# umautobots/LONER

Hardware: AMD Instinct MI355X
Metric: training rays/sec (higher is better)
Workload: dtype f32

## Files before the change

loner_amd/csrc/lnr_density.hip:

```cpp
#include <stdlib.h>

#include "lnr_density_api.h"
#include <vector>
#include <cstdlib>
#include <cstdio>

#include <mutex>
#include <unordered_map>

typedef float f32x4 __attribute__((ext_vector_type(4)));

#define LNR_ENC_BWD_MAX_BPG 2048

namespace {
struct WsNote { uint64_t layout; uint32_t epoch; bool ovf_zero; };
std::mutex g_ws_mutex;
std::unordered_map<const void*, WsNote> g_ws_notes;

uint64_t layout_signature(const LnrNetSpec* spec, int64_t cap) {
    uint64_t h = 1469598103934665603ull;
    auto mix = [&](const void* p, size_t n) { const unsigned char* b = (const unsigned char*)p; for (size_t i = 0; i < n; ++i) { h ^= b[i]; h *= 1099511628211ull; } };
    mix(spec, sizeof(LnrNetSpec));
    mix(&cap, sizeof(cap));
    return h;
}
void ws_bound_locked() { if (g_ws_notes.size() > 64) g_ws_notes.clear(); }
void ws_touch(const void* ws, uint64_t layout) {
    std::lock_guard<std::mutex> lock(g_ws_mutex);
    ws_bound_locked();
    auto it = g_ws_notes.find(ws);
    if (it == g_ws_notes.end()) g_ws_notes[ws] = WsNote{layout, 0u, false};
    else if (it->second.layout != layout) { it->second.layout = layout; it->second.ovf_zero = false; }
}
void ws_backward_begin(const void* ws, uint64_t layout, int* epoch, bool* clear) {
    std::lock_guard<std::mutex> lock(g_ws_mutex);
    ws_bound_locked();
    WsNote& n = g_ws_notes[ws];
    if (n.layout != layout) { n.layout = layout; n.ovf_zero = false; }
    *clear = !n.ovf_zero;
    n.ovf_zero = false;
    n.epoch = n.epoch >= 0x7FFFFFF0u ? 1u : n.epoch + 1u;
    if (n.epoch == 1u) *clear = true;
    *epoch = (int)n.epoch;
}
void ws_backward_done(const void* ws) {
    std::lock_guard<std::mutex> lock(g_ws_mutex);
    auto it = g_ws_notes.find(ws);
    if (it != g_ws_notes.end()) it->second.ovf_zero = true;
}
void ws_forget(const void* ws) {
    std::lock_guard<std::mutex> lock(g_ws_mutex);
    g_ws_notes.erase(ws);
}
}

#define LNR_SLAB_GROUPS 16
__device__ __forceinline__ void slab_fold_block(const float* __restrict__ slabs, int n_slabs, int n_mlp, float* __restrict__ grad, int overwrite, int block) {
    __shared__ float part[LNR_SLAB_GROUPS][64];
    const int px = threadIdx.x & 63, gy = threadIdx.x >> 6;
    const int i = block * 64 + px;
    const int per = (n_slabs + LNR_SLAB_GROUPS - 1) / LNR_SLAB_GROUPS;
    int b = gy * per;
    const int b_end = min(n_slabs, b + per);
    float s0 = 0.0f, s1 = 0.0f, s2 = 0.0f, s3 = 0.0f;
    if (i < n_mlp) {
        for (; b + 3 < b_end; b += 4) {
            s0 += slabs[(size_t)b * n_mlp + i]; s1 += slabs[(size_t)(b + 1) * n_mlp + i];
            s2 += slabs[(size_t)(b + 2) * n_mlp + i]; s3 += slabs[(size_t)(b + 3) * n_mlp + i];
        }
        for (; b < b_end; ++b) s0 += slabs[(size_t)b * n_mlp + i];
    }
    part[gy][px] = (s0 + s1) + (s2 + s3);
    __syncthreads();
    if (gy == 0 && i < n_mlp) {
        float s = 0.0f;
#pragma unroll
        for (int k = 0; k < LNR_SLAB_GROUPS; ++k) s += part[k][px];
        grad[i] = overwrite ? s : grad[i] + s;
    }
}
__global__ void __launch_bounds__(64 * LNR_SLAB_GROUPS)
reduce_slabs_kernel(const float* __restrict__ slabs, int n_slabs, int n_mlp, float* __restrict__ grad, int overwrite) {
    slab_fold_block(slabs, n_slabs, n_mlp, grad, overwrite, (int)blockIdx.x);
}

template <int PAIR>
__device__ __forceinline__ void reduce_one(long long* acc, uint2 r, uint32_t base) {
    if (PAIR) {
        uint32_t pi; float v0, v1;
        lnr_unpack_pair(r, pi, v0, v1);
        unsigned long long* a = reinterpret_cast<unsigned long long*>(acc) + 2 * pi;
        if (__builtin_expect(__builtin_fmaxf(__builtin_fabsf(v0), __builtin_fabsf(v1)) < 256.0f, 1)) {
            atomicAdd(a, (unsigned long long)lnr_to_fix_small(v0));
            atomicAdd(a + 1, (unsigned long long)lnr_to_fix_small(v1));
        } else {
            atomicAdd(a, (unsigned long long)lnr_to_fix(v0));
            atomicAdd(a + 1, (unsigned long long)lnr_to_fix(v1));
        }
    } else {
        const float v = __uint_as_float(r.y);
        if (v != 0.0f) atomicAdd(reinterpret_cast<unsigned long long*>(&acc[r.x - base]), (unsigned long long)lnr_to_fix(v));
    }
}
__device__ __forceinline__ void reduce_xpair(long long* acc, const LnrXRec& r) {
    uint32_t pi, t; float a0, a1, fx;
    lnr_unpack_xpair(r, pi, t, a0, a1, fx);
    const uint32_t pj = pi ^ ((2u << t) - 1u);
    long long q[4];
    lnr_xpair_fix(a0, a1, fx, q);
    unsigned long long* a = reinterpret_cast<unsigned long long*>(acc);
    atomicAdd(a + 2 * pi, (unsigned long long)q[0]);
    atomicAdd(a + 2 * pi + 1, (unsigned long long)q[1]);
    atomicAdd(a + 2 * pj, (unsigned long long)q[2]);
    atomicAdd(a + 2 * pj + 1, (unsigned long long)q[3]);
}

#ifdef LNR_PHASE_TIMING
__device__ unsigned long long lnr_reduce_phase_cycles[LNR_N_PHASES];
#endif
#define RED_SLICE (1 << LNR_SLICE_SHIFT)

typedef uint32_t red_u32x3 __attribute__((ext_vector_type(3), aligned(4)));
typedef uint32_t red_u32x4 __attribute__((ext_vector_type(4)));
__device__ __forceinline__ LnrXRec load_xrec_stream(const char* p) {
    const red_u32x3 v = __builtin_nontemporal_load(reinterpret_cast<const red_u32x3*>(p));
    LnrXRec r; r.a = v.x; r.b = v.y; r.c = v.z;
    return r;
}
__device__ __forceinline__ uint4 load_rec2_stream(const uint4* p) {
    const red_u32x4 v = __builtin_nontemporal_load(reinterpret_cast<const red_u32x4*>(p));
    return make_uint4(v.x, v.y, v.z, v.w);
}

template <int PAIR, int RED_U>
__device__ __forceinline__ void reduce_regions(long long* acc, const int* __restrict__ wave_counts, const char* __restrict__ wave_regions, int n_regions,
                                               uint32_t region_bytes, bool xp, uint32_t base, int lane) {
    for (int r0 = 0; r0 < n_regions; r0 += 64) {
        const int nq = min(64, n_regions - r0);
        const int my_n = lane < nq ? wave_counts[r0 + lane] : 0;
        const char* round_regions = wave_regions + (size_t)r0 * region_bytes;
        if (xp) {
            LnrXRec cur[RED_U][2], nxt[RED_U][2];
            auto loadx = [&](int q0, LnrXRec out[RED_U][2]) {
#pragma unroll
                for (int u = 0; u < RED_U; ++u) {
                    const int q = q0 + u < nq ? q0 + u : nq - 1;
                    const int n = __builtin_amdgcn_readlane(my_n, q);
                    const char* rg = round_regions + (size_t)q * region_bytes;
                    out[u][0] = load_xrec_stream(rg + (lane < n ? lane : 0) * 12);
                    out[u][1] = load_xrec_stream(rg + (lane + 64 < n ? lane + 64 : 0) * 12);
                }
            };
            loadx(0, nxt);
            for (int q0 = 0; q0 < nq; q0 += RED_U) {
#pragma unroll
                for (int u = 0; u < RED_U; ++u) { cur[u][0] = nxt[u][0]; cur[u][1] = nxt[u][1]; }
                if (q0 + RED_U < nq) loadx(q0 + RED_U, nxt);
#pragma unroll
                for (int u = 0; u < RED_U; ++u) {
                    const int n = q0 + u < nq ? __builtin_amdgcn_readlane(my_n, q0 + u < 64 ? q0 + u : 63) : 0;
                    if (lane < n) reduce_xpair(acc, cur[u][0]);
                    if (lane + 64 < n) reduce_xpair(acc, cur[u][1]);
                }
            }
            unsigned long long more = __ballot(my_n > 128);
            while (more) {
                const int q = __builtin_ctzll(more);
                more &= more - 1ull;
                const int n = __builtin_amdgcn_readlane(my_n, q);
                const char* rg = round_regions + (size_t)q * region_bytes;
                for (int off = 128; off < n; off += 64 * 4) {
                    LnrXRec r[4];
#pragma unroll
                    for (int u = 0; u < 4; ++u) { const int k = off + 64 * u + lane; r[u] = load_xrec_stream(rg + (size_t)(k < n ? k : n - 1) * 12); }
#pragma unroll
                    for (int u = 0; u < 4; ++u) if (off + 64 * u + lane < n) reduce_xpair(acc, r[u]);
                }
            }
            continue;
        }
        uint4 cur[RED_U], nxt[RED_U];
        auto load4 = [&](int q0, uint4 out[RED_U]) {
#pragma unroll
            for (int u = 0; u < RED_U; ++u) {
                const int q = q0 + u < nq ? q0 + u : nq - 1;
                const int n = __builtin_amdgcn_readlane(my_n, q);
                out[u] = load_rec2_stream(reinterpret_cast<const uint4*>(round_regions + (size_t)q * region_bytes) + (2 * lane < n ? lane : 0));
            }
        };
        load4(0, nxt);
        for (int q0 = 0; q0 < nq; q0 += RED_U) {
#pragma unroll
            for (int u = 0; u < RED_U; ++u) cur[u] = nxt[u];
            if (q0 + RED_U < nq) load4(q0 + RED_U, nxt);
#pragma unroll
            for (int u = 0; u < RED_U; ++u) {
                const int n = q0 + u < nq ? __builtin_amdgcn_readlane(my_n, q0 + u < 64 ? q0 + u : 63) : 0;
                if (2 * lane < n) reduce_one<PAIR>(acc, make_uint2(cur[u].x, cur[u].y), base);
                if (2 * lane + 1 < n) reduce_one<PAIR>(acc, make_uint2(cur[u].z, cur[u].w), base);
            }
        }
        unsigned long long more = __ballot(my_n > 128);
        while (more) {
            const int q = __builtin_ctzll(more);
            more &= more - 1ull;
            const int n = __builtin_amdgcn_readlane(my_n, q);
            const uint2* rg = reinterpret_cast<const uint2*>(round_regions + (size_t)q * region_bytes);
            for (int off = 128; off < n; off += 128 * 4) {
                uint4 r[4];
#pragma unroll
                for (int u = 0; u < 4; ++u) { const int k = off + 128 * u + 2 * lane; r[u] = load_rec2_stream(reinterpret_cast<const uint4*>(rg) + (k < n ? k : 0) / 2); }
#pragma unroll
                for (int u = 0; u < 4; ++u) {
                    const int k = off + 128 * u + 2 * lane;
                    if (k < n) reduce_one<PAIR>(acc, make_uint2(r[u].x, r[u].y), base);
                    if (k + 1 < n) reduce_one<PAIR>(acc, make_uint2(r[u].z, r[u].w), base);
                }
            }
        }
    }
}

struct RedLevel { uint64_t lo, hi; };
__device__ __forceinline__ RedLevel red_level(const LnrNetSpec& spec, int l) {
    RedLevel r;
    r.lo = (uint64_t)spec.level_offset[l] * spec.n_features;
    r.hi = r.lo + (uint64_t)spec.level_size[l] * spec.n_features;
    return r;
}

template <int PAIR, int RED_U, int MINW>
__global__ void __launch_bounds__(1024, MINW)
table_grad_reduce_split_kernel(const LnrNetSpec spec, const void* __restrict__ regions_v, const RegionPlan plan, const int* __restrict__ counts, int bpg,
                               int maxo, long long* __restrict__ ovf) {
    extern __shared__ long long acc[];
    constexpr int slice = RED_SLICE, shift = LNR_SLICE_SHIFT;
    int b = blockIdx.x, l = 0, span = 0;
    int64_t my_ovf = 0;
    RedLevel lv;
    for (;; ++l) {
        lv = red_level(spec, l);
        span = (int)(((lv.hi - 1) >> shift) - (lv.lo >> shift)) + 1;
        const int n = plan.split[l] > 1 ? span * plan.split[l] : 0;
        if (b < n) break;
        b -= n;
        my_ovf += (int64_t)(lv.hi - lv.lo);
    }
    const int parts = plan.split[l], local = b / parts, part = b % parts;
    const uint32_t base = ((uint32_t)(lv.lo >> shift) + (uint32_t)local) << shift;
    const uint32_t region_bytes = plan.bytes[l];
    if (region_bytes == 0u) return;
#pragma unroll
    for (int i = threadIdx.x; i < slice; i += 1024) acc[i] = 0ll;
    __syncthreads();
    const int lane = threadIdx.x & 63, wave = __builtin_amdgcn_readfirstlane(threadIdx.x >> 6);
    const int per_part = (bpg + parts - 1) / parts, part_first = part * per_part, part_n = min(per_part, bpg - part_first);
    const int per_wave = (part_n + 15) / 16, first = part_first + wave * per_wave, n_regions = min(per_wave, part_first + part_n - first);
    if (n_regions > 0)
        reduce_regions<PAIR, RED_U>(acc, counts + ((size_t)l * maxo + local) * bpg + first,
                                    reinterpret_cast<const char*>(regions_v) + plan.off[l] + ((size_t)local * bpg + first) * (size_t)region_bytes, n_regions,
                                    region_bytes, PAIR && plan.xp[l] != 0, base, lane);
    __syncthreads();
#pragma unroll
    for (int k = 0; k < slice / 1024; ++k) {
        const int i = threadIdx.x + k * 1024;
        const uint64_t gi = (uint64_t)base + i;
        const long long q = acc[i];
        if (q != 0ll && gi >= lv.lo && gi < lv.hi) atomicAdd(reinterpret_cast<unsigned long long*>(ovf + my_ovf + (int64_t)(gi - lv.lo)), (unsigned long long)q);
    }
}

template <int PAIR, int RED_U, int MINW>
__global__ void __launch_bounds__(1024, MINW)
table_grad_reduce2_kernel(const LnrNetSpec spec, const void* __restrict__ regions_v, const RegionPlan plan, const int* __restrict__ counts, int bpg,
                          int maxo, long long* __restrict__ ovf, const int* __restrict__ ovf_flag, int epoch, float* __restrict__ grad_table,
                          int64_t n_table_floats, int overwrite, const float* __restrict__ slabs, int n_slabs, int n_mlp, float* __restrict__ grad_mlp) {
    extern __shared__ long long acc[];
    const int slab_blocks = slabs != nullptr ? (n_mlp + 63) / 64 : 0;
    const int owner_blocks = (int)gridDim.x - slab_blocks;
    if ((int)blockIdx.x >= owner_blocks) {
        slab_fold_block(slabs, n_slabs, n_mlp, grad_mlp, overwrite, (int)blockIdx.x - owner_blocks);
        return;
    }
    const int o = owner_blocks - 1 - (int)blockIdx.x;
    constexpr int slice = RED_SLICE, shift = LNR_SLICE_SHIFT;
    const uint32_t base = (uint32_t)o << shift;
    PHASE_INIT();
#pragma unroll
    for (int i = threadIdx.x; i < slice; i += 1024) acc[i] = 0ll;
    __syncthreads();
    PHASE(0);
    const int lane = threadIdx.x & 63, wave = __builtin_amdgcn_readfirstlane(threadIdx.x >> 6);
    constexpr int nwaves = 16;
    int64_t ovf_off = 0;
    for (int l = 0; l < spec.n_levels; ++l) {
        const RedLevel lv = red_level(spec, l);
        const uint64_t lo = lv.lo, hi = lv.hi;
        const int64_t my_ovf = ovf_off;
        ovf_off += (int64_t)(hi - lo);
        if (hi <= base || lo >= (uint64_t)base + slice) continue;
        if (plan.split[l] > 1 || ovf_flag[l] == epoch) {
            long long v[slice / 1024];
#pragma unroll
            for (int k = 0; k < slice / 1024; ++k) {
                const uint64_t gi = (uint64_t)base + threadIdx.x + k * 1024;
                v[k] = (gi >= lo && gi < hi) ? ovf[my_ovf + (int64_t)(gi - lo)] : 0ll;
            }
#pragma unroll
            for (int k = 0; k < slice / 1024; ++k) {
                if (v[k] != 0ll) {
                    acc[threadIdx.x + k * 1024] += v[k];
                    ovf[my_ovf + (int64_t)((uint64_t)base + threadIdx.x + k * 1024 - lo)] = 0ll;
                }
            }
            __syncthreads();
            PHASE(1);
        }
        const int local = o - (int)(lo >> shift);
        if (local < 0 || local >= maxo) continue;
        const uint32_t region_bytes = plan.bytes[l];
        if (region_bytes == 0u || plan.split[l] > 1) continue;
        const int per_wave = (bpg + nwaves - 1) / nwaves;
        const int first = wave * per_wave;
        const int n_regions = min(per_wave, bpg - first);
        if (n_regions > 0)
            reduce_regions<PAIR, RED_U>(acc, counts + ((size_t)l * maxo + local) * bpg + first,
                                        reinterpret_cast<const char*>(regions_v) + plan.off[l] + ((size_t)local * bpg + first) * (size_t)region_bytes, n_regions,
                                        region_bytes, PAIR && plan.xp[l] != 0, base, lane);
        PHASE(3);
    }
    __syncthreads();
    PHASE(5);
    {
        float g[slice / 1024];
#pragma unroll
        for (int k = 0; k < slice / 1024; ++k) {
            const int64_t gi = (int64_t)base + threadIdx.x + k * 1024;
            g[k] = (!overwrite && gi < n_table_floats) ? grad_table[gi] : 0.0f;
        }
#pragma unroll
        for (int k = 0; k < slice / 1024; ++k) {
            const int64_t gi = (int64_t)base + threadIdx.x + k * 1024;
            const long long q = acc[threadIdx.x + k * 1024];
            if (gi < n_table_floats && (overwrite || q != 0ll)) grad_table[gi] = g[k] + (float)((double)q * (1.0 / (double)LNR_FIX_SCALE));
        }
    }
    PHASE(6);
    PHASE_FLUSH(lnr_reduce_phase_cycles, 0);
}

struct Layout {
    int64_t m_pad;
    int n_groups, bpg, maxo, shift, nown, n_split;
    RegionPlan plan;
    size_t off_status, off_feat, off_wide, off_dfeat, off_dxl, off_dpts, off_rayacc, off_slabs, off_ovf, off_counts, off_regions, total;
};

static size_t align256(size_t v) { return (v + 255) & ~(size_t)255; }

static Layout make_layout(const LnrNetSpec* spec, int64_t n_points, const DensityRoute& route) {
    Layout L;
    L.m_pad = (n_points + 63) / 64 * 64;
    if (L.m_pad < 64) L.m_pad = 64;
#ifndef LNR_PLANE_SKEW
#define LNR_PLANE_SKEW 1088
#endif
    if (LNR_PLANE_SKEW > 0 && (L.m_pad * (int64_t)sizeof(float)) % 65536 == 0) L.m_pad += LNR_PLANE_SKEW;
    const bool hash = spec->encoding == LNR_ENC_HASHGRID;
    L.n_groups = hash ? spec->n_levels : 1;
    L.shift = LNR_SLICE_SHIFT;
    const int64_t n_table = spec->n_params - spec->n_mlp_params;
    L.nown = (int)((n_table + (1 << L.shift) - 1) >> L.shift);
    int64_t bpg = (n_points + LNR_ENC_BWD_BLOCK * LNR_BATCHES_PER_WG - 1) / (LNR_ENC_BWD_BLOCK * LNR_BATCHES_PER_WG);
    if (bpg < 1) bpg = 1;
    if (bpg > LNR_ENC_BWD_MAX_BPG) bpg = LNR_ENC_BWD_MAX_BPG;
    bpg = (bpg + 3) & ~(int64_t)3;
    L.bpg = (int)bpg;
    L.maxo = 1;
    size_t ovf_total = 0;
    uint64_t region_total = 0;
    for (int l = 0; l < LNR_MAX_LEVELS; ++l) { L.plan.off[l] = 0; L.plan.bytes[l] = 0; L.plan.xp[l] = 0; L.plan.split[l] = 1; L.plan.binned[l] = 0; }
    L.n_split = 0;
    if (hash) {
        const int F = spec->n_features;
        for (int pass = 0; pass < 2; ++pass) {
            if (pass == 1 && region_total <= LNR_REGION_BUDGET) break;
            const double shrink = pass == 0 ? 1.0 : (double)LNR_REGION_BUDGET / (double)region_total;
            region_total = 0; ovf_total = 0; L.maxo = 1; L.n_split = 0;
            for (int l = 0; l < spec->n_levels; ++l) {
                ovf_total += (size_t)spec->level_size[l] * F;
                const uint64_t lo = (uint64_t)spec->level_offset[l] * F, hi = lo + (uint64_t)spec->level_size[l] * F;
                const int span = (int)(((hi - 1) >> L.shift) - (lo >> L.shift)) + 1;
                if (span > L.maxo) L.maxo = span;
                const bool xp = lnr_level_can_use_xpairs(*spec, l, LNR_XPAIR_SCALE_MIN);
                L.plan.xp[l] = xp ? 1 : 0;
                double r = (double)n_points * 8.0 * (F >= 2 ? F / 2.0 : 1.0) / (double)span / (double)L.bpg;
                if (xp) r *= 0.5;
                else if (spec->level_scale[l] < LNR_COMBINE_SCALE_MAX) r *= LNR_COMBINE_FILL;
                const double recs = (r * (xp ? LNR_REGION_HEADROOM_XP : LNR_REGION_HEADROOM) + LNR_REGION_SLACK) * shrink;
                uint64_t bytes = (uint64_t)(recs * (xp ? 12.0 : 8.0));
                const double bin_fill = (double)LNR_ENC_BWD_BLOCK * 8.0 * (xp ? 0.5 * 12.0 : 8.0) / (double)span;
                const bool binned = F >= 2 && spec->level_hashed[l] != 0 && span <= LNR_BIN_MAX_OWNERS && bin_fill <= 0.5 * LNR_BIN_BYTES + 8.0 &&
                                    LNR_ENC_BWD_BLOCK == 512 && shrink == 1.0;
                L.plan.binned[l] = binned ? 1 : 0;
                if (binned) bytes += LNR_BIN_BYTES + 128;
                bytes = (bytes + 255u) & ~(uint64_t)255u;
                int parts = spec->level_hashed[l] == 0 ? LNR_REDUCE_SPLIT : 1;
                while (parts > 1 && L.bpg / parts < 16) parts >>= 1;
                L.plan.split[l] = (uint8_t)(parts < 1 ? 1 : parts);
// ... 247 lines not shown
    ws_forget(workspace);
    if (hipMemsetAsync(workspace, 0, LNR_WORKSPACE_STATUS_BYTES, (hipStream_t)stream) != hipSuccess) {
        lnr_set_error("lnr_density_workspace_init: hipMemsetAsync failed");
        return LNR_ERR_LAUNCH;
    }
    return LNR_OK;
}

extern "C" int lnr_density_workspace_release(void* workspace) {
    LNR_REQUIRE(workspace != nullptr, "lnr_density_workspace_release: null workspace");
    ws_forget(workspace);
    return LNR_OK;
}

extern "C" int lnr_density_forward(const LnrNetSpec* spec, const float* params, const float* pts, int64_t n_points,
                                   const float* rays, const float* z, int32_t n_rays, int32_t n_samples,
                                   const int32_t* n_rays_dev, float* sigma, void* workspace, size_t workspace_bytes, void* stream) {
    int rc = check_spec(spec, "lnr_density_forward");
    if (rc) return rc;
    if (n_points == 0 && (pts != nullptr || n_rays == 0)) return LNR_OK;
    PointSrc src; MlpPoints mp;
    rc = make_src(&src, &mp, pts, n_points, rays, z, n_rays, n_samples, n_rays_dev, "lnr_density_forward");
    if (rc) return rc;
    const int64_t cap = mp.n_points;
    if (cap == 0) return LNR_OK;
    LNR_REQUIRE(params && sigma && workspace, "lnr_density_forward: null params/sigma/workspace");
    const DensityRoute route = lnr_route(spec, cap, false);
    const Layout L = make_layout(spec, cap, route);
    LNR_REQUIRE(L.m_pad * (spec->n_features > 4 ? spec->n_features : 4) < (1ll << 30),
                "lnr_density_forward: too many points per call for 32-bit plane offsets (padded n_points * max(n_features, 4) must be < 2^30)");
    if (workspace_bytes < L.off_dfeat) {
        lnr_set_error("lnr_density_forward: workspace %zu < %zu (lnr_density_workspace_forward)", workspace_bytes, L.off_dfeat);
        return LNR_ERR_WORKSPACE;
    }
    if (route.kind == LNR_ROUTE_UNSUPPORTED) return route_unsupported(spec, route, "lnr_density_forward");
    hipStream_t st = (hipStream_t)stream;
    ws_touch(workspace, layout_signature(spec, cap));
    float* feat = (float*)((char*)workspace + L.off_feat);
    mp.clip_flag = reinterpret_cast<int32_t*>((char*)workspace + L.off_status) + LNR_STATUS_CLIPPED;
    if (!route.fused_enc) {
        LnrProfScope prof("encode_forward", st);
        rc = lnr_encode_forward(spec, params, &src, cap, feat, L.m_pad, spec->precision == LNR_PREC_F16, st);
    }
    if (rc) return rc;
    LNR_CHECK_LAUNCH("lnr_density_forward(encode)");
    LnrProfScope prof_mlp("mlp_forward", st);
    const MlpArgs a{spec, &route, params, feat, L.m_pad, &mp, sigma, nullptr, nullptr, nullptr, 0, 0, &src, nullptr, (char*)workspace + L.off_wide, st};
    const char* what;
    switch (route.kind) {
        case LNR_ROUTE_WIDE: rc = lnr_mlp_fwd_wide(a); what = "lnr_density_forward(mlp 256 x n)"; break;
        case LNR_ROUTE_F16_FAST: case LNR_ROUTE_F16_FREQ: case LNR_ROUTE_F16_GEN: rc = lnr_mlp_fwd_f16(a); what = "lnr_density_forward(mlp f16)"; break;
        case LNR_ROUTE_BF3: rc = lnr_mlp_fwd_bf3(a); what = "lnr_density_forward(mlp bf16x3)"; break;
        default: rc = mlp_fwd_ht(a); what = "lnr_density_forward(mlp)"; break;
    }
    if (rc) return rc;
    LNR_CHECK_LAUNCH(what);
    return LNR_OK;
}

extern "C" int lnr_density_backward(const LnrNetSpec* spec, const float* params, const float* pts, int64_t n_points,
                                    const float* rays, const float* z, int32_t n_rays, int32_t n_samples,
                                    const int32_t* n_rays_dev, const float* d_sigma, float* grad_params, float* d_pts, float* d_rays,
                                    int32_t reuse_features, int32_t flags, void* workspace, size_t workspace_bytes, void* input_grad_event,
                                    void* stream) {
    int rc = check_spec(spec, "lnr_density_backward");
    if (rc) return rc;
    auto empty_batch = [&]() -> int {
        if (input_grad_event != nullptr && hipEventRecord((hipEvent_t)input_grad_event, (hipStream_t)stream) != hipSuccess) {
            lnr_set_error("lnr_density_backward: hipEventRecord failed");
            return LNR_ERR_LAUNCH;
        }
        return LNR_OK;
    };
    if (n_points == 0 && (pts != nullptr || n_rays == 0)) return empty_batch();
    PointSrc src; MlpPoints mp;
    rc = make_src(&src, &mp, pts, n_points, rays, z, n_rays, n_samples, n_rays_dev, "lnr_density_backward");
    if (rc) return rc;
    const int64_t cap = mp.n_points;
    if (cap == 0) return empty_batch();
    LNR_REQUIRE(params && d_sigma && workspace, "lnr_density_backward: null argument");
    LNR_REQUIRE(grad_params || d_pts || d_rays, "lnr_density_backward: nothing to compute (no grad_params, d_pts or d_rays)");
    const DensityRoute route = lnr_route(spec, cap, true);
    const Layout L = make_layout(spec, cap, route);
    LNR_REQUIRE(L.m_pad * (spec->n_features > 4 ? spec->n_features : 4) < (1ll << 30),
                "lnr_density_backward: too many points per call for 32-bit plane offsets (padded n_points * max(n_features, 4) must be < 2^30)");
    if (workspace_bytes < L.total) {
        lnr_set_error("lnr_density_backward: workspace %zu < %zu (lnr_density_workspace)", workspace_bytes, L.total);
        return LNR_ERR_WORKSPACE;
    }
    if (route.kind == LNR_ROUTE_UNSUPPORTED) return route_unsupported(spec, route, "lnr_density_backward");
    hipStream_t st = (hipStream_t)stream;
    char* ws = (char*)workspace;
    float* feat = (float*)(ws + L.off_feat);
    float* dfeat = (float*)(ws + L.off_dfeat);
    float* dxl = (float*)(ws + L.off_dxl);
    float* slabs = (float*)(ws + L.off_slabs);
    long long* ovf = (long long*)(ws + L.off_ovf);
    int* counts = (int*)(ws + L.off_counts);
    void* regions = (void*)(ws + L.off_regions);
    const bool hash = spec->encoding == LNR_ENC_HASHGRID;
    RegionPlan rplan = L.plan;
    if (flags & LNR_BWD_TABLE_ATOMICS)
        for (int l = 0; l < LNR_MAX_LEVELS; ++l) rplan.bytes[l] = 0;
    if (!(flags & LNR_BWD_BINS))
        for (int l = 0; l < LNR_MAX_LEVELS; ++l) rplan.binned[l] = 0;
    const bool want_grad = grad_params != nullptr;

    const bool fused_freq = route.fused_enc;
    if (!reuse_features && !fused_freq) {
        LnrProfScope prof("encode_forward", st);
        rc = lnr_encode_forward(spec, params, &src, cap, feat, L.m_pad, spec->precision == LNR_PREC_F16, st);
        if (rc) return rc;
        LNR_CHECK_LAUNCH("lnr_density_backward(encode)");
    }
    LNR_REQUIRE(!(d_rays && pts), "lnr_density_backward: d_rays needs the rays form");
    LNR_REQUIRE(!(d_rays && d_pts), "lnr_density_backward: pass d_pts or d_rays, not both");
    const bool ray_accum = d_rays != nullptr && hash && (n_samples % 64 == 0);
    float* d_pts_eff = d_pts;
    if (d_rays && !ray_accum) d_pts_eff = (float*)(ws + L.off_dpts);
    const int want_dfeat = ((hash && want_grad) || d_pts_eff != nullptr || ray_accum) ? 1 : 0;
    {
    LnrProfScope prof("mlp_backward", st);
    const MlpArgs a{spec, &route, params, feat, L.m_pad, &mp, nullptr, d_sigma, dfeat, slabs, want_dfeat, want_grad ? 1 : 0, &src, d_pts_eff, ws + L.off_wide, st};
    switch (route.kind) {
        case LNR_ROUTE_WIDE: rc = lnr_mlp_bwd_wide(a); break;
        case LNR_ROUTE_F16_FAST: case LNR_ROUTE_F16_FREQ: case LNR_ROUTE_F16_GEN: rc = lnr_mlp_bwd_f16(a); break;
        case LNR_ROUTE_BF3: rc = lnr_mlp_bwd_bf3(a); break;
        case LNR_ROUTE_REGS: rc = mlp_bwd_regs(a); break;
        default: rc = mlp_bwd_ht(a); break;
    }
    }
    if (rc) return rc;
    LNR_CHECK_LAUNCH("lnr_density_backward(mlp)");
    float* grad_table = want_grad ? grad_params + spec->n_mlp_params : nullptr;
    int* ovf_flag = reinterpret_cast<int32_t*>(ws + L.off_status) + LNR_STATUS_OVF_LEVEL0;
    int epoch = 0;
    const bool uses_ovf = hash && want_grad;
    if (uses_ovf) {
        bool clear = false;
        ws_backward_begin(workspace, layout_signature(spec, cap), &epoch, &clear);
        if (clear && (hipMemsetAsync(ovf, 0, L.off_counts - L.off_ovf, st) != hipSuccess ||
                      hipMemsetAsync(ovf_flag, 0, LNR_MAX_LEVELS * sizeof(int32_t), st) != hipSuccess)) {
            lnr_set_error("lnr_density_backward: hipMemsetAsync failed");
            return LNR_ERR_LAUNCH;
        }
    } else {
        ws_touch(workspace, layout_signature(spec, cap));
    }
    const bool fold_in_reduce = want_grad && hash && L.nown > 0 && !(flags & LNR_BWD_DEFER_WEIGHT_FOLD);
    ReduceCtx rctx{spec, regions, counts, ovf, ovf_flag, epoch, grad_table, rplan, L.bpg, L.maxo, L.shift, spec->n_params - spec->n_mlp_params,
                   (flags & LNR_BWD_TABLE_ATOMICS) ? 0 : L.n_split, (flags & LNR_BWD_OVERWRITE_GRAD) ? 1 : 0,
                   fold_in_reduce ? slabs : nullptr, route.n_slabs, spec->n_mlp_params, grad_params};
    if (want_dfeat && !fused_freq) {
        rc = lnr_encode_backward(spec, params, &src, cap, dfeat, dxl, L.m_pad, grad_table, want_grad ? regions : nullptr, &rplan, counts,
                                 L.bpg, L.maxo, L.shift,
                                 ovf, ovf_flag, epoch, d_pts_eff, ray_accum ? d_rays : nullptr, (long long*)(ws + L.off_rayacc), (flags & LNR_BWD_BINS_W8) != 0, st);
        if (rc) return rc;
        LNR_CHECK_LAUNCH("lnr_density_backward(encode backward)");
    }
    if (d_rays && !ray_accum) {
        rc = lnr_points_grad_to_rays(d_pts_eff, z, n_rays, n_rays_dev, n_samples, d_rays, stream);
        if (rc) return rc;
    }
    if (input_grad_event != nullptr && hipEventRecord((hipEvent_t)input_grad_event, st) != hipSuccess) {
        lnr_set_error("lnr_density_backward: hipEventRecord failed");
        return LNR_ERR_LAUNCH;
    }
    if (!want_grad) return LNR_OK;
    if (want_dfeat) {
        if (hash && (flags & LNR_BWD_REPORT_REGIONS)) {
            int64_t live = cap;
            int32_t nr = 0;
            if (n_rays_dev && hipStreamSynchronize(st) == hipSuccess && hipMemcpy(&nr, n_rays_dev, sizeof(nr), hipMemcpyDeviceToHost) == hipSuccess) live = (int64_t)nr * n_samples;
            report_regions(spec, L, rplan, counts, dfeat, live, st);
        }
    }
    if (hash && L.nown > 0) {
        rc = launch_table_reduce(rctx, L.nown, st);
        if (rc) return rc;
        LNR_CHECK_LAUNCH("lnr_density_backward(table reduce)");
        ws_backward_done(workspace);
#ifdef LNR_PHASE_TIMING
        if (getenv("LNR_PHASE_TIMING")) {
            static const char* names[LNR_N_PHASES] = {"zero LDS", "overflow fold", "-", "records", "-", "final barrier", "write-out"};
            unsigned long long h[LNR_N_PHASES];
            if (lnr_phase_fetch(HIP_SYMBOL(lnr_reduce_phase_cycles), h, LNR_N_PHASES, st)) lnr_phase_print("table_grad_reduce", names, h);
        }
#endif
    }
    if ((flags & LNR_BWD_DEFER_WEIGHT_FOLD) || fold_in_reduce) return LNR_OK;
    const int n_mlp = spec->n_mlp_params;
    LnrProfScope prof_slabs("reduce_slabs", st);
    hipLaunchKernelGGL(reduce_slabs_kernel, dim3(lnr_div_up(n_mlp, 64)), dim3(64 * LNR_SLAB_GROUPS), 0, st, slabs, route.n_slabs, n_mlp, grad_params,
                       (flags & LNR_BWD_OVERWRITE_GRAD) ? 1 : 0);
    LNR_CHECK_LAUNCH("lnr_density_backward(reduce)");
    return LNR_OK;
}

extern "C" int lnr_density_fold_weight_grads(const LnrNetSpec* spec, int64_t n_points, float* grad_params, void* workspace,
                                             size_t workspace_bytes, int32_t flags, void* stream) {
    int rc = check_spec(spec, "lnr_density_fold_weight_grads");
    if (rc) return rc;
    LNR_REQUIRE(grad_params && workspace && n_points > 0, "lnr_density_fold_weight_grads: bad argument");
    const DensityRoute route = lnr_route(spec, n_points, true);
    const Layout L = make_layout(spec, n_points, route);
    LNR_REQUIRE(workspace_bytes >= L.total, "lnr_density_fold_weight_grads: workspace too small");
    if (route.kind == LNR_ROUTE_UNSUPPORTED) return route_unsupported(spec, route, "lnr_density_fold_weight_grads");
    const int n_mlp = spec->n_mlp_params;
    hipStream_t st = (hipStream_t)stream;
    LnrProfScope prof_slabs("reduce_slabs", st);
    hipLaunchKernelGGL(reduce_slabs_kernel, dim3(lnr_div_up(n_mlp, 64)), dim3(64 * LNR_SLAB_GROUPS), 0, st,
                       (const float*)((const char*)workspace + L.off_slabs), route.n_slabs, n_mlp, grad_params, (flags & LNR_BWD_OVERWRITE_GRAD) ? 1 : 0);
    LNR_CHECK_LAUNCH("lnr_density_fold_weight_grads");
    return LNR_OK;
}

__global__ void selftest_mfma_kernel(float* out) {
    const int lane = threadIdx.x;
    const int i = lane & 15, k = lane >> 4;
    const float a = (float)(i * 7 + k * 3 + 1) * 0.25f;
    const float b = (float)((lane & 15) * 5 - k * 11 + 2) * 0.5f;
    f32x4 d = f32x4{0.0f, 0.0f, 0.0f, 0.0f};
    d = __builtin_amdgcn_mfma_f32_16x16x4f32(a, b, d, 0, 0, 0);
    float err = 0.0f;
    const int j = lane & 15;
    for (int r = 0; r < 4; ++r) {
        const int row = 4 * (lane >> 4) + r;
        float ref = 0.0f;
        for (int kk = 0; kk < 4; ++kk) ref += ((float)(row * 7 + kk * 3 + 1) * 0.25f) * ((float)(j * 5 - kk * 11 + 2) * 0.5f);
        err = fmaxf(err, fabsf(ref - d[r]));
    }
    err = wave_max(err);
    if (lane == 0) out[0] = err;
}

extern "C" int lnr_selftest_mfma(float* out, void* stream) {
    LNR_REQUIRE(out != nullptr, "lnr_selftest_mfma: null out");
    hipLaunchKernelGGL(selftest_mfma_kernel, dim3(1), dim3(64), 0, (hipStream_t)stream, out);
    lnr_selftest_mfma_f16(out, (hipStream_t)stream);
    lnr_selftest_mfma_bf3(out, (hipStream_t)stream);
    LNR_CHECK_LAUNCH("lnr_selftest_mfma");
    return LNR_OK;
}
```

loner_amd/csrc/lnr_density_api.h:

```cpp
#pragma once
#include "lnr_common.h"

#define LNR_DENSITY_BLOCK 256
#define LNR_DENSITY_MAX_BLOCKS 1024
#define LNR_LDS_LIMIT (160 * 1024)

struct PointSrc {
    const float* pts;
    const float* rays;
    const float* z;
    int32_t n_samples;
    int64_t n_points;
    int32_t n_rays;
    const int32_t* n_rays_dev;
};

#define LNR_BWD_MAX_BLOCKS 512
#define LNR_SLICE_SHIFT 13
#define LNR_REGION_BUDGET (24ull << 30)
#define LNR_COMBINE_SCALE_MAX 3000.0f
#define LNR_COMBINE_FILL 1.0
#ifndef LNR_REGION_HEADROOM
#define LNR_REGION_HEADROOM 2.0
#endif
#ifndef LNR_REGION_SLACK
#define LNR_REGION_SLACK 64.0
#endif
#ifndef LNR_REGION_HEADROOM_XP
#define LNR_REGION_HEADROOM_XP LNR_REGION_HEADROOM
#endif
#ifndef LNR_ENC_BWD_BLOCK
#define LNR_ENC_BWD_BLOCK 512
#endif
#ifndef LNR_BATCHES_PER_WG
#define LNR_BATCHES_PER_WG 4
#endif
#define LNR_REDUCE_SPLIT 32
#define LNR_FIX_SCALE 4398046511104.0f
#define LNR_BIN_BYTES 1024
#define LNR_BIN_MAX_OWNERS 64
#ifndef LNR_XPAIR_SCALE_MIN
#define LNR_XPAIR_SCALE_MIN 3000.0f
#endif

__device__ __forceinline__ long long lnr_to_fix_small(float v) {
    const double d = __builtin_fma((double)v, 4398046511104.0, 6755399441055744.0);
    return __double_as_longlong(d) - 0x4338000000000000ll;
}
__device__ __forceinline__ long long lnr_to_fix(float v) {
    if (__builtin_expect(__builtin_fabsf(v) < 256.0f, 1)) return lnr_to_fix_small(v);
    return __float2ll_rn(v * LNR_FIX_SCALE);
}

static_assert(LNR_SLICE_SHIFT == 13, "pair records hold a 12-bit pair index: 8192-float owner slices");
__host__ __device__ __forceinline__ uint32_t lnr_pack26(float v) {
    uint32_t u;
    memcpy(&u, &v, 4);
    u += 0x1Fu + ((u >> 6) & 1u);
    return u >> 6;
}
__device__ __forceinline__ uint2 lnr_pack_pair(uint32_t pair_idx, float v0, float v1) {
    const uint32_t a = lnr_pack26(v0), b = lnr_pack26(v1);
    return make_uint2((b << 12) | (pair_idx & 0xFFFu), (a << 6) | (b >> 20));
}
__device__ __forceinline__ void lnr_unpack_pair(uint2 r, uint32_t& pair_idx, float& v0, float& v1) {
    pair_idx = r.x & 0xFFFu;
    v0 = __uint_as_float(r.y & 0xFFFFFFC0u);
    v1 = __uint_as_float(((r.y & 0x3Fu) << 26) | ((r.x >> 6) & 0x03FFFFC0u));
}

struct LnrXRec { uint32_t a, b, c; };
__device__ __forceinline__ LnrXRec lnr_pack_xpair(uint32_t pair_idx, uint32_t t, float a0, float a1, float fx) {
    const uint32_t p0 = lnr_pack26(a0), p1 = lnr_pack26(a1);
    uint32_t fb;
    memcpy(&fb, &fx, 4);
    fb = (fb + 8u) >> 4;
    LnrXRec r;
    r.a = (pair_idx & 0xFFFu) | ((t & 0xFu) << 12) | ((p0 >> 10) << 16);
    r.b = ((p0 & 0x3FFu) << 22) | (p1 >> 4);
    r.c = ((p1 & 0xFu) << 28) | (fb & 0x0FFFFFFFu);
    return r;
}
__device__ __forceinline__ void lnr_unpack_xpair(const LnrXRec& r, uint32_t& pair_idx, uint32_t& t, float& a0, float& a1, float& fx) {
    pair_idx = r.a & 0xFFFu;
    t = (r.a >> 12) & 0xFu;
    a0 = __uint_as_float((((r.a >> 16) << 10) | (r.b >> 22)) << 6);
    a1 = __uint_as_float((((r.b & 0x3FFFFFu) << 4) | (r.c >> 28)) << 6);
    fx = __uint_as_float((r.c & 0x0FFFFFFFu) << 4);
}
__device__ __forceinline__ void lnr_xpair_fix(float a0, float a1, float fx, long long q[4]) {
    const float gx = 1.0f - fx;
    if (__builtin_expect(__builtin_fmaxf(__builtin_fabsf(a0), __builtin_fabsf(a1)) < 256.0f, 1)) {
        q[0] = lnr_to_fix_small(gx * a0); q[1] = lnr_to_fix_small(gx * a1); q[2] = lnr_to_fix_small(fx * a0); q[3] = lnr_to_fix_small(fx * a1);
    } else {
        q[0] = __float2ll_rn(gx * a0 * LNR_FIX_SCALE); q[1] = __float2ll_rn(gx * a1 * LNR_FIX_SCALE);
        q[2] = __float2ll_rn(fx * a0 * LNR_FIX_SCALE); q[3] = __float2ll_rn(fx * a1 * LNR_FIX_SCALE);
    }
}
static inline bool lnr_level_can_use_xpairs(const LnrNetSpec& s, int l, float scale_min) {
    const uint32_t size = s.level_size[l];
    return s.n_features == 2 && s.level_hashed[l] != 0 && (size & (size - 1u)) == 0u && s.level_scale[l] >= scale_min &&
           ((s.level_offset[l] * 2u) & ((1u << LNR_SLICE_SHIFT) - 1u)) == 0u;
}

__host__ __device__ inline int lnr_w_stride(int cols) { return cols + 4; }
__host__ __device__ inline int lnr_w_lds_floats(int H, int in_dim, int n_hidden, bool with_first) {
    return (with_first ? H * lnr_w_stride(in_dim) : 0) + (n_hidden - 1) * H * lnr_w_stride(H) + 16 * H;
}

struct DensityRoute {
    int kind;
    int lds_misfit;
    int grid;
    int waves;
    int w_lds;
    int dw64;
    size_t lds;
    int n_slabs;
    int f16_part;
    bool fused_enc;
    size_t wide_bytes;
};

struct MlpPoints {
    int64_t n_points;
    const int32_t* n_rays_dev;
    int32_t n_rays, n_samples;
    int32_t* clip_flag;
};

struct MlpArgs {
    const LnrNetSpec* spec;
    const DensityRoute* route;
    const float* params;
    const float* feat;
    int64_t m_pad;
    const MlpPoints* pt;
    float* sigma;
    const float* d_sigma;
    float* dfeat;
    float* slabs;
    int want_dfeat, want_dw;
    const PointSrc* src;
    float* d_pts;
    void* planes;
    hipStream_t st;
};

#define LNR_DECLARE_HT(HT) int lnr_mlp_fwd_ht##HT(const MlpArgs& a); int lnr_mlp_bwd_ht##HT(const MlpArgs& a);
#define LNR_DECLARE_REGS(HT, NH) int lnr_mlp_bwd_regs_ht##HT##_nh##NH(const MlpArgs& a);
LNR_DECLARE_REGS(4, 1) LNR_DECLARE_REGS(4, 2) LNR_DECLARE_REGS(4, 3)
LNR_DECLARE_REGS(8, 1) LNR_DECLARE_REGS(8, 2) LNR_DECLARE_REGS(8, 3)
LNR_DECLARE_REGS(16, 1)
LNR_DECLARE_HT(1)
LNR_DECLARE_HT(2)
LNR_DECLARE_HT(4)
LNR_DECLARE_HT(8)
LNR_DECLARE_HT(16)

struct LevelList {
    int n;
    int lv[LNR_MAX_LEVELS];
    int slab_off[LNR_MAX_LEVELS];
};

struct RegionPlan {
    uint64_t off[LNR_MAX_LEVELS];
    uint32_t bytes[LNR_MAX_LEVELS];
    uint8_t xp[LNR_MAX_LEVELS];
    uint8_t split[LNR_MAX_LEVELS];
    uint8_t binned[LNR_MAX_LEVELS];
};

int lnr_encode_forward(const LnrNetSpec* spec, const float* params, const PointSrc* src, int64_t cap_points, float* feat,
                       int64_t m_pad, bool half_planes, hipStream_t st);

bool lnr_f16_supported(const LnrNetSpec* spec);
bool lnr_f16_fast_class(const LnrNetSpec* spec);
bool lnr_f16_fused_freq(const LnrNetSpec* spec);
int lnr_mlp_fwd_f16(const MlpArgs& a);
int lnr_mlp_bwd_f16(const MlpArgs& a);
int lnr_selftest_mfma_f16(float* out, hipStream_t st);
bool lnr_bf3_class(const LnrNetSpec* spec, int64_t n_points);
int lnr_mlp_fwd_bf3(const MlpArgs& a);
int lnr_mlp_bwd_bf3(const MlpArgs& a);
int lnr_selftest_mfma_bf3(float* out, hipStream_t st);
bool lnr_wide_class(const LnrNetSpec* spec);
size_t lnr_wide_workspace(const LnrNetSpec* spec, int64_t n_points);
int lnr_mlp_fwd_wide(const MlpArgs& a);
int lnr_mlp_bwd_wide(const MlpArgs& a);
// ... 5 lines not shown
```

loner_amd/csrc/lnr_density_bf3.hip:

```cpp
#include "lnr_f16_common.h"

typedef __bf16 bf16x8 __attribute__((ext_vector_type(8)));
typedef __bf16 bf16x2 __attribute__((ext_vector_type(2)));

#define BF3_TS 36
#ifndef LNR_BF3_FWD_OCC
#define LNR_BF3_FWD_OCC 3
#endif

struct Frag3 { u32x4 t[3]; };

__device__ __forceinline__ void bf3_split_pair(float x, float y, uint32_t& p0, uint32_t& p1, uint32_t& p2) {
    p0 = __builtin_bit_cast(uint32_t, bf16x2{(__bf16)x, (__bf16)y});
    asm volatile("" : "+v"(p0));
    float rx = x - __uint_as_float(p0 << 16), ry = y - __uint_as_float(p0 & 0xFFFF0000u);
    p1 = __builtin_bit_cast(uint32_t, bf16x2{(__bf16)rx, (__bf16)ry});
    asm volatile("" : "+v"(p1));
    rx -= __uint_as_float(p1 << 16);
    ry -= __uint_as_float(p1 & 0xFFFF0000u);
    p2 = __builtin_bit_cast(uint32_t, bf16x2{(__bf16)rx, (__bf16)ry});
}
__device__ __forceinline__ void bf3_split8(const float v[8], Frag3& f) {
#pragma unroll
    for (int q = 0; q < 4; ++q) {
        uint32_t p0, p1, p2;
        bf3_split_pair(v[2 * q], v[2 * q + 1], p0, p1, p2);
        f.t[0][q] = p0; f.t[1][q] = p1; f.t[2][q] = p2;
    }
}
#define BF3_M(a, b, acc) __builtin_amdgcn_mfma_f32_16x16x32_bf16(__builtin_bit_cast(bf16x8, a), __builtin_bit_cast(bf16x8, b), acc, 0, 0, 0)
#define BF3_FOR_TERMS(X) X(0, 2) X(2, 0) X(1, 1) X(0, 1) X(1, 0) X(0, 0)
__device__ __forceinline__ f32x4 bf3_mfma6(const Frag3& a, const Frag3& b, f32x4 acc) {
    acc = BF3_M(a.t[0], b.t[2], acc);
    acc = BF3_M(a.t[2], b.t[0], acc);
    acc = BF3_M(a.t[1], b.t[1], acc);
    acc = BF3_M(a.t[0], b.t[1], acc);
    acc = BF3_M(a.t[1], b.t[0], acc);
    acc = BF3_M(a.t[0], b.t[0], acc);
    return acc;
}

__device__ __forceinline__ void bf3_load_x2(const float* __restrict__ fb, uint32_t plane_bytes, uint32_t m_even, float x[2][8]) {
#pragma unroll
    for (int i = 0; i < 8; ++i) {
        const float2 v = ld32<float2>(fb, (uint32_t)i * plane_bytes + m_even * 4u);
        x[0][i] = v.x; x[1][i] = v.y;
    }
}

template <int HT>
__global__ void __launch_bounds__(LNR_DENSITY_BLOCK, LNR_BF3_FWD_OCC)
mlp_forward_bf3_kernel(const float* __restrict__ params, const float* __restrict__ feat, int64_t m_pad, int64_t n_points,
                       const int32_t* __restrict__ n_rays_dev, int n_rays, int n_samples, float* __restrict__ sigma, int32_t* __restrict__ clip_flag) {
    constexpr int H = 16 * HT;
    const int lane = threadIdx.x & 63, wave = threadIdx.x >> 6, nw = blockDim.x >> 6;
    const int c = lane & 15, g = lane >> 4;
    Frag3 wa[HT]; float wo[HT][4];
#pragma unroll
    for (int jt = 0; jt < HT; ++jt) {
        float v[8];
#pragma unroll
        for (int i = 0; i < 8; ++i) v[i] = params[(16 * jt + c) * 32 + 8 * g + i];
        bf3_split8(v, wa[jt]);
#pragma unroll
        for (int r = 0; r < 4; ++r) wo[jt][r] = params[H * 32 + 16 * jt + 4 * g + r];
    }
    const int64_t M = live_samples(n_points, n_rays_dev, n_rays, n_samples);
    const int64_t n_tiles = M > 0 ? (M + 31) / 32 : 0;
    const int64_t stride = (int64_t)gridDim.x * nw;
    int64_t tile = (int64_t)blockIdx.x * nw + wave;
    if (tile >= n_tiles) return;
    const float* fb = feat + (size_t)(8 * g) * m_pad;
    const uint32_t plane_bytes = (uint32_t)m_pad * 4u;
    float cur[2][8], nxt[2][8];
    bf3_load_x2(fb, plane_bytes, (uint32_t)(tile * 32 + 2 * c), cur);
    bf3_load_x2(fb, plane_bytes, (uint32_t)((tile + stride < n_tiles ? tile + stride : tile) * 32 + 2 * c), nxt);
    while (tile < n_tiles) {
        const int64_t nt = tile + stride, nt2 = nt + stride;
        float nx2[2][8];
        bf3_load_x2(fb, plane_bytes, (uint32_t)((nt2 < n_tiles ? nt2 : tile) * 32 + 2 * c), nx2);
        __builtin_amdgcn_sched_barrier(0);
        Frag3 xb0, xb1;
        bf3_split8(cur[0], xb0);
        bf3_split8(cur[1], xb1);
        f32x4 Z0[HT], Z1[HT];
#pragma unroll
        for (int jt = 0; jt < HT; ++jt) { Z0[jt] = f32x4{0.0f, 0.0f, 0.0f, 0.0f}; Z1[jt] = f32x4{0.0f, 0.0f, 0.0f, 0.0f}; }
#define BF3_X(IA, IB)                                                                          \
    _Pragma("unroll") for (int jt = 0; jt < HT; ++jt) { Z0[jt] = BF3_M(wa[jt].t[IA], xb0.t[IB], Z0[jt]); Z1[jt] = BF3_M(wa[jt].t[IA], xb1.t[IB], Z1[jt]); }
        BF3_FOR_TERMS(BF3_X)
#undef BF3_X
        float p0 = 0.0f, p1 = 0.0f;
#pragma unroll
        for (int jt = 0; jt < HT; ++jt)
#pragma unroll
            for (int r = 0; r < 4; ++r) { p0 += wo[jt][r] * fmaxf(Z0[jt][r], 0.0f); p1 += wo[jt][r] * fmaxf(Z1[jt][r], 0.0f); }
        p0 += __shfl_xor(p0, 16, 64); p1 += __shfl_xor(p1, 16, 64);
        p0 += __shfl_xor(p0, 32, 64); p1 += __shfl_xor(p1, 32, 64);
        const int64_t m = tile * 32 + 2 * c;
        if (g == 0 && m < M) {
            p0 = finite_or_clipped<false>(p0, clip_flag);
            if (m + 1 < M) { p1 = finite_or_clipped<false>(p1, clip_flag); *reinterpret_cast<float2*>(sigma + m) = make_float2(p0, p1); }
            else sigma[m] = p0;
        }
#pragma unroll
        for (int t = 0; t < 2; ++t)
#pragma unroll
            for (int i = 0; i < 8; ++i) { cur[t][i] = nxt[t][i]; nxt[t][i] = nx2[t][i]; }
        tile = nt;
    }
}

template <int HT>
struct Bf3Lds {
    static constexpr int H = 16 * HT, KB = (HT + 1) / 2, NW = LNR_DENSITY_BLOCK / 64;
    static constexpr size_t N_MLP = (size_t)H * 32 + 16 * H;
    static constexpr size_t OFF_T = N_MLP * sizeof(float);
    static constexpr size_t OFF_WA = OFF_T + (size_t)NW * H * BF3_TS * sizeof(float);
    static constexpr size_t OFF_WT = OFF_WA + (size_t)3 * HT * 64 * 16;
    static constexpr size_t BYTES = OFF_WT + (size_t)3 * 2 * KB * 64 * 16;
};

template <int HT>
__global__ void __launch_bounds__(LNR_DENSITY_BLOCK, 2)
mlp_backward_bf3_kernel(const float* __restrict__ params, int n_mlp, const float* __restrict__ feat, int64_t m_pad, int64_t n_points,
                        const int32_t* __restrict__ n_rays_dev, int n_rays, int n_samples, const float* __restrict__ d_sigma,
                        float* __restrict__ dfeat, float* __restrict__ slabs, int want_dfeat) {
    extern __shared__ __attribute__((aligned(16))) float smem[];
    using L = Bf3Lds<HT>;
    constexpr int H = 16 * HT, KB = L::KB;
    const int nw = blockDim.x >> 6;
    const int lane = threadIdx.x & 63, wave = threadIdx.x >> 6;
    const int c = lane & 15, g = lane >> 4;
    float* dW = smem;
    float* T = reinterpret_cast<float*>(reinterpret_cast<char*>(smem) + L::OFF_T) + wave * (H * BF3_TS);
    u32x4* WA = reinterpret_cast<u32x4*>(reinterpret_cast<char*>(smem) + L::OFF_WA);
    u32x4* WT = reinterpret_cast<u32x4*>(reinterpret_cast<char*>(smem) + L::OFF_WT);
    for (int i = threadIdx.x; i < n_mlp; i += blockDim.x) dW[i] = 0.0f;
    for (int job = wave; job < HT + 2 * KB; job += nw) {
        float v[8];
        if (job < HT) {
#pragma unroll
            for (int i = 0; i < 8; ++i) v[i] = params[(16 * job + c) * 32 + 8 * g + i];
        } else {
            const int it = (job - HT) / KB, kb = (job - HT) % KB;
#pragma unroll
            for (int i = 0; i < 8; ++i) {
                const int n = 32 * kb + (i < 4 ? 4 * g + i : 16 + 4 * g + (i - 4));
                v[i] = n < H ? params[n * 32 + 16 * it + c] : 0.0f;
            }
        }
        Frag3 f;
        bf3_split8(v, f);
#pragma unroll
        for (int t3 = 0; t3 < 3; ++t3) {
            if (job < HT) WA[(t3 * HT + job) * 64 + lane] = f.t[t3];
            else WT[(t3 * 2 * KB + (job - HT)) * 64 + lane] = f.t[t3];
        }
    }
    float wo[HT][4];
#pragma unroll
    for (int jt = 0; jt < HT; ++jt)
#pragma unroll
        for (int r = 0; r < 4; ++r) wo[jt][r] = params[H * 32 + 16 * jt + 4 * g + r];
    __syncthreads();
    f32x4 dW1_acc[HT][2];
    float dWo_acc[HT][4];
#pragma unroll
    for (int jt = 0; jt < HT; ++jt) {
        dW1_acc[jt][0] = f32x4{0.0f, 0.0f, 0.0f, 0.0f};
        dW1_acc[jt][1] = f32x4{0.0f, 0.0f, 0.0f, 0.0f};
#pragma unroll
        for (int r = 0; r < 4; ++r) dWo_acc[jt][r] = 0.0f;
    }

    const int64_t M = live_samples(n_points, n_rays_dev, n_rays, n_samples);
    const int64_t n_tiles = M > 0 ? (M + 31) / 32 : 0;
    const int64_t stride = (int64_t)gridDim.x * nw;
    const uint32_t plane_bytes = (uint32_t)m_pad * 4u;
    const float* fb = feat + (size_t)(8 * g) * m_pad;
    const float* fc = feat + (size_t)c * m_pad;
    float* db = dfeat + (size_t)(4 * g) * m_pad;
    int64_t tile = (int64_t)blockIdx.x * nw + wave;
    float xcur[2][8], dcur[2];
    auto load_front = [&](int64_t tl, float (&x)[2][8], float (&ds)[2]) {
        const int64_t m = tl * 32 + 2 * c;
        bf3_load_x2(fb, plane_bytes, (uint32_t)m, x);
        const float v0 = d_sigma[m < M ? m : M - 1], v1 = d_sigma[m + 1 < M ? m + 1 : M - 1];
        ds[0] = m < M ? v0 : 0.0f;
        ds[1] = m + 1 < M ? v1 : 0.0f;
    };
    float xnxt[2][8], dnxt[2];
    if (tile < n_tiles) { load_front(tile, xcur, dcur); load_front(tile + stride < n_tiles ? tile + stride : tile, xnxt, dnxt); }
    while (tile < n_tiles) {
        const int64_t nt = tile + stride;
        const int64_t nt2 = nt + stride;
        float xnx2[2][8], dnx2[2];
        load_front(nt2 < n_tiles ? nt2 : tile, xnx2, dnx2);
        const bool any = (dcur[0] != 0.0f) | (dcur[1] != 0.0f);
        if (__ballot(any) == 0ull) {
            if (want_dfeat) {
#pragma unroll
                for (int k = 0; k < 8; ++k)
                    st32<float2>(db, (uint32_t)(16 * (k >> 2) + (k & 3)) * plane_bytes + (uint32_t)(tile * 32 + 2 * c) * 4u, make_float2(0.0f, 0.0f));
            }
        } else {
            float xraw[2][8];
#pragma unroll
            for (int it = 0; it < 2; ++it) {
                const uint32_t off = (uint32_t)(16 * it) * plane_bytes + (uint32_t)(tile * 32 + 8 * g) * 4u;
                const float4 a = ld32<float4>(fc, off), b = ld32<float4>(fc, off + 16u);
                xraw[it][0] = a.x; xraw[it][1] = a.y; xraw[it][2] = a.z; xraw[it][3] = a.w;
                xraw[it][4] = b.x; xraw[it][5] = b.y; xraw[it][6] = b.z; xraw[it][7] = b.w;
            }
            Frag3 xf[2];
            bf3_split8(xcur[0], xf[0]);
            bf3_split8(xcur[1], xf[1]);
            int wl = lane;
            asm volatile("" : "+v"(wl));
            float dz[HT][2][4];
#pragma unroll
            for (int jt = 0; jt < HT; ++jt) {
                Frag3 wa;
#pragma unroll
                for (int t3 = 0; t3 < 3; ++t3) wa.t[t3] = WA[(t3 * HT + jt) * 64 + wl];
                f32x4 Z0 = f32x4{0.0f, 0.0f, 0.0f, 0.0f}, Z1 = f32x4{0.0f, 0.0f, 0.0f, 0.0f};
#define BF3_X(IA, IB) Z0 = BF3_M(wa.t[IA], xf[0].t[IB], Z0); Z1 = BF3_M(wa.t[IA], xf[1].t[IB], Z1);
                BF3_FOR_TERMS(BF3_X)
#undef BF3_X
#pragma unroll
                for (int r = 0; r < 4; ++r) {
                    dWo_acc[jt][r] += dcur[0] * fmaxf(Z0[r], 0.0f) + dcur[1] * fmaxf(Z1[r], 0.0f);
                    dz[jt][0][r] = Z0[r] > 0.0f ? dcur[0] * wo[jt][r] : 0.0f;
                    dz[jt][1][r] = Z1[r] > 0.0f ? dcur[1] * wo[jt][r] : 0.0f;
                    *reinterpret_cast<float2*>(T + (16 * jt + 4 * g + r) * BF3_TS + 2 * c) = make_float2(dz[jt][0][r], dz[jt][1][r]);
                }
            }
            Frag3 xs[2];
            bf3_split8(xraw[0], xs[0]);
            bf3_split8(xraw[1], xs[1]);
#pragma unroll
            for (int it = 0; it < 2; ++it)
#pragma unroll
                for (int t3 = 0; t3 < 3; ++t3) asm volatile("" : "+v"(xs[it].t[t3]));
            if (want_dfeat) {
                f32x4 D[2][2];
#pragma unroll
                for (int t = 0; t < 2; ++t) {
                    D[t][0] = f32x4{0.0f, 0.0f, 0.0f, 0.0f}; D[t][1] = f32x4{0.0f, 0.0f, 0.0f, 0.0f};
#pragma unroll
                    for (int kb = 0; kb < KB; ++kb) {
                        constexpr bool odd = (HT & 1) != 0;
                        float v[8];
#pragma unroll
                        for (int i = 0; i < 4; ++i) {
                            v[i] = dz[2 * kb][t][i];
                            v[4 + i] = (odd && 2 * kb + 1 >= HT) ? 0.0f : dz[(2 * kb + 1 < HT) ? 2 * kb + 1 : 2 * kb][t][i];
                        }
                        Frag3 b;
                        bf3_split8(v, b);
#pragma unroll
                        for (int it = 0; it < 2; ++it) {
                            Frag3 a;
#pragma unroll
                            for (int t3 = 0; t3 < 3; ++t3) a.t[t3] = WT[((t3 * 2 + it) * KB + kb) * 64 + wl];
                            D[t][it] = bf3_mfma6(a, b, D[t][it]);
                        }
                    }
                }
#pragma unroll
                for (int it = 0; it < 2; ++it)
#pragma unroll
                    for (int r = 0; r < 4; ++r)
                        st32<float2>(db, (uint32_t)(16 * it + r) * plane_bytes + (uint32_t)(tile * 32 + 2 * c) * 4u, make_float2(D[0][it][r], D[1][it][r]));
            }
            __builtin_amdgcn_fence(__ATOMIC_RELEASE, "wavefront");
            __builtin_amdgcn_wave_barrier();
            __builtin_amdgcn_fence(__ATOMIC_ACQUIRE, "wavefront");
#pragma unroll
            for (int jt = 0; jt < HT; ++jt) {
                const float4 a0 = *reinterpret_cast<const float4*>(T + (16 * jt + c) * BF3_TS + 8 * g);
                const float4 a1 = *reinterpret_cast<const float4*>(T + (16 * jt + c) * BF3_TS + 8 * g + 4);
                const float v[8] = {a0.x, a0.y, a0.z, a0.w, a1.x, a1.y, a1.z, a1.w};
                Frag3 a;
                bf3_split8(v, a);
#define BF3_X(IA, IB) dW1_acc[jt][0] = BF3_M(a.t[IA], xs[0].t[IB], dW1_acc[jt][0]); dW1_acc[jt][1] = BF3_M(a.t[IA], xs[1].t[IB], dW1_acc[jt][1]);
                BF3_FOR_TERMS(BF3_X)
#undef BF3_X
            }
            __builtin_amdgcn_fence(__ATOMIC_RELEASE, "wavefront");
            __builtin_amdgcn_wave_barrier();
        }
#pragma unroll
        for (int t = 0; t < 2; ++t) {
#pragma unroll
            for (int i = 0; i < 8; ++i) { xcur[t][i] = xnxt[t][i]; xnxt[t][i] = xnx2[t][i]; }
            dcur[t] = dnxt[t]; dnxt[t] = dnx2[t];
        }
        tile = nt;
    }
    float* dW1 = dW;
    float* dWo = dW + H * 32;
    for (int turn = 0; turn < nw; ++turn) {
        if (wave == turn) {
#pragma unroll
            for (int jt = 0; jt < HT; ++jt) {
#pragma unroll
                for (int it = 0; it < 2; ++it)
#pragma unroll
                    for (int r = 0; r < 4; ++r) dW1[(16 * jt + 4 * g + r) * 32 + 16 * it + c] += dW1_acc[jt][it][r];
#pragma unroll
                for (int r = 0; r < 4; ++r) {
                    float v = dWo_acc[jt][r];
                    v += __shfl_xor(v, 1, 64); v += __shfl_xor(v, 2, 64); v += __shfl_xor(v, 4, 64); v += __shfl_xor(v, 8, 64);
                    if (c == 0) dWo[16 * jt + 4 * g + r] += v;
                }
            }
        }
        __syncthreads();
    }
    float* slab = slabs + (size_t)blockIdx.x * n_mlp;
    for (int i = threadIdx.x; i < n_mlp; i += blockDim.x) slab[i] = dW[i];
}

bool lnr_bf3_class(const LnrNetSpec* spec, int64_t n_points) {
    return spec->precision == LNR_PREC_F32 && spec->encoding == LNR_ENC_HASHGRID && spec->activation == LNR_ACT_RELU && spec->n_hidden == 1 &&
           spec->in_dim == 32 && spec->enc_dim == 32 && spec->n_neurons <= 64 && (spec->n_neurons == 16 || spec->n_neurons == 32 || spec->n_neurons == 64) &&
           n_points <= (1ll << 25) - 2048;
}

int lnr_mlp_fwd_bf3(const MlpArgs& a) {
    const MlpPoints* pt = a.pt;
    const dim3 grid((unsigned)a.route->grid), block(LNR_DENSITY_BLOCK);
#define LNR_BF3_FWD(HT) hipLaunchKernelGGL(mlp_forward_bf3_kernel<HT>, grid, block, 0, a.st, a.params, a.feat, a.m_pad, pt->n_points, pt->n_rays_dev, pt->n_rays, pt->n_samples, a.sigma, pt->clip_flag)
    switch (a.spec->n_neurons / 16) {
        case 1: LNR_BF3_FWD(1); break;
        case 2: LNR_BF3_FWD(2); break;
        default: LNR_BF3_FWD(4); break;
    }
#undef LNR_BF3_FWD
    return LNR_OK;
}

int lnr_mlp_bwd_bf3(const MlpArgs& a) {
    const MlpPoints* pt = a.pt;
    const dim3 grid((unsigned)a.route->grid), block(LNR_DENSITY_BLOCK);
#define LNR_BF3_BWD(HT)                                                                                                          \
    do {                                                                                                                         \
        int rc_ = f16_set_lds(mlp_backward_bf3_kernel<HT>, Bf3Lds<HT>::BYTES, "lnr_density_backward");                           \
        if (rc_) return rc_;                                                                                                     \
        hipLaunchKernelGGL(mlp_backward_bf3_kernel<HT>, grid, block, Bf3Lds<HT>::BYTES, a.st, a.params, a.spec->n_mlp_params, a.feat, a.m_pad, \
                           pt->n_points, pt->n_rays_dev, pt->n_rays, pt->n_samples, a.d_sigma, a.dfeat, a.slabs, a.want_dfeat); \
    } while (0)
    switch (a.spec->n_neurons / 16) {
        case 1: LNR_BF3_BWD(1); break;
        case 2: LNR_BF3_BWD(2); break;
        default: LNR_BF3_BWD(4); break;
    }
#undef LNR_BF3_BWD
    return LNR_OK;
}

__global__ void selftest_mfma_bf3_kernel(float* out) {
    const int lane = threadIdx.x;
    const int c = lane & 15, g = lane >> 4;
    auto A = [](int i, int k) { return (float)((i * 397 + k * 1013) % 4093 - 2046) * 0.015625f; };
    auto B = [](int k, int j) { return (float)((k * 743 - j * 211) % 3571 - 1785) * 0.015625f; };
    float av[8], bv[8];
    for (int i = 0; i < 8; ++i) { av[i] = A(c, 8 * g + i); bv[i] = B(8 * g + i, c); }
    Frag3 a, b;
    bf3_split8(av, a);
    bf3_split8(bv, b);
    const f32x4 d = bf3_mfma6(a, b, f32x4{0.0f, 0.0f, 0.0f, 0.0f});
    float err = 0.0f;
    for (int r = 0; r < 4; ++r) {
        double ref = 0.0;
        for (int k = 0; k < 32; ++k) ref += (double)A(4 * g + r, k) * (double)B(k, c);
        err = fmaxf(err, fabsf((float)(ref - (double)d[r])));
    }
    const float x = 1.0f + (float)(lane * 2654435 % 8388607) * 1.1920929e-7f;
    uint32_t p0, p1, p2;
    bf3_split_pair(x, -x, p0, p1, p2);
    const float back = (__uint_as_float(p0 << 16) + __uint_as_float(p1 << 16)) + __uint_as_float(p2 << 16);
    const float backy = (__uint_as_float(p0 & 0xFFFF0000u) + __uint_as_float(p1 & 0xFFFF0000u)) + __uint_as_float(p2 & 0xFFFF0000u);
    if (back != x || backy != -x) err = 1e9f;
    err = wave_max(err);
    if (lane == 0) out[2] = err;
}

int lnr_selftest_mfma_bf3(float* out, hipStream_t st) {
    hipLaunchKernelGGL(selftest_mfma_bf3_kernel, dim3(1), dim3(64), 0, st, out);
    return LNR_OK;
}
```

loner_amd/csrc/lnr_encode.hip:

```cpp
#include "lnr_encoding.h"
#include <cstdio>
#include <cstdlib>

#define ENC_BLOCK 256

__device__ __forceinline__ bool level_slot(int bpg, int n_slots, bool xcd_affine, int& slot, int& chunk) {
    if (xcd_affine) {
        const int r = (int)(blockIdx.x >> 3);
        slot = (int)(blockIdx.x & 7u) + 8 * (r / bpg);
        chunk = r % bpg;
    } else {
        slot = (int)blockIdx.x / bpg;
        chunk = (int)blockIdx.x % bpg;
    }
    return slot < n_slots;
}
#ifndef LNR_XCD_AFFINE_MAX_POINTS
#define LNR_XCD_AFFINE_MAX_POINTS (1 << 19)
#endif
static inline bool lnr_xcd_affine(int n_slots, int64_t n_points, bool forward) {
    const bool on = forward && n_points <= LNR_XCD_AFFINE_MAX_POINTS;
    return on && n_slots > 0 && n_slots % 8 == 0;
}

// ... 189 lines not shown
    const int64_t M = live_points(src);
    const int64_t M16 = (M + 15) / 16 * 16;
    for (int64_t m = (int64_t)chunk * ENC_BLOCK + threadIdx.x; m < M16; m += (int64_t)bpg * ENC_BLOCK) {
        float out[4] = {0.0f, 0.0f, 0.0f, 0.0f};
        if (m < M) {
            float x[3];
            load_unit_point(src, m, x);
            freq_features4(spec, x, 4 * group, out);
        }
#pragma unroll
        for (int r = 0; r < 4; ++r)
            if (4 * group + r < spec.enc_dim) feat[(size_t)(4 * group + r) * m_pad + m] = out[r];
    }
}

__global__ void __launch_bounds__(ENC_BLOCK)
freq_forward_h16_kernel(const LnrNetSpec spec, const PointSrc src, uint32_t* __restrict__ pairs, int64_t m_pad, int bpg) {
    typedef _Float16 h2 __attribute__((ext_vector_type(2)));
    const int dim = blockIdx.x / bpg, chunk = blockIdx.x % bpg;
    const int nf = spec.n_frequencies;
    const int64_t M = live_points(src);
    const int64_t M32 = (M + 31) / 32 * 32;
    for (int64_t m = (int64_t)chunk * ENC_BLOCK + threadIdx.x; m < M32; m += (int64_t)bpg * ENC_BLOCK) {
        float xv = 0.0f;
        const bool live = m < M;
        if (live) {
            float x[3];
            load_unit_point(src, m, x);
            xv = dim == 0 ? x[0] : (dim == 1 ? x[1] : x[2]);
        }
        for (int f = 0; f < nf; ++f) {
            const float mult = __uint_as_float((uint32_t)(127 + f) << 23);
            const float ph = lnr_mul_rn(lnr_mul_rn(xv, mult), LNR_PI_F);
            float s, c;
            sincos_f32(ph, &s, &c);
            const float h = lnr_add_rn(ph, LNR_PI_2_F);
            const float bb = lnr_add_rn(h, -ph);
            const float e = lnr_add_rn(lnr_add_rn(ph, -lnr_add_rn(h, -bb)), lnr_add_rn(LNR_PI_2_F, -bb));
            const float d = 4.371139000186243e-8f - e;
            const float c2 = __builtin_fmaf(-d, s, c);
            const uint32_t v = live ? __builtin_bit_cast(uint32_t, h2{(_Float16)s, (_Float16)c2}) : 0u;
            pairs[(size_t)(dim * nf + f) * (size_t)m_pad + (size_t)m] = v;
        }
    }
}

struct EncSink {
    float* grad_table;
    long long* ovf;
    void* regions;
    RegionPlan plan;
    int* counts;
    int maxo, shift;
    int xcd_affine;
    int* ovf_flag;
    int epoch;
    float combine_scale_max;
};

struct RunMask { bool take1, take2, take4, take8; };

struct RunMul { float m1, m2, m4, m8; };
__device__ __forceinline__ RunMul run_multipliers(const RunMask& k) {
    return RunMul{k.take1 ? 1.0f : 0.0f, k.take2 ? 1.0f : 0.0f, k.take4 ? 1.0f : 0.0f, k.take8 ? 1.0f : 0.0f};
}
template <int N>
__device__ __forceinline__ void row_run_sum_n(float (&v)[N], const RunMul& m) {
#pragma unroll
    for (int i = 0; i < N; ++i) v[i] = __builtin_fmaf(row_down_f<1>(v[i]), m.m1, v[i]);
#pragma unroll
    for (int i = 0; i < N; ++i) v[i] = __builtin_fmaf(row_down_f<2>(v[i]), m.m2, v[i]);
#pragma unroll
    for (int i = 0; i < N; ++i) v[i] = __builtin_fmaf(row_down_f<4>(v[i]), m.m4, v[i]);
#pragma unroll
    for (int i = 0; i < N; ++i) v[i] = __builtin_fmaf(row_down_f<8>(v[i]), m.m8, v[i]);
}

__device__ __forceinline__ void cell_runs(const Cell& c, int lane, bool& head, RunMask& run) {
    const int c16 = lane & 15;
    const int k1 = (int)(c.b[0] | (c.b[1] << 16)), k2 = (int)c.b[2];
    const int p1 = row_up_i<1>(k1), p2 = row_up_i<1>(k2);
    head = (c16 == 0) | (p1 != k1) | (p2 != k2);
    int seg = head ? 1 : 0;
    int t;
    t = row_up_i<1>(seg); if (c16 >= 1) seg += t;
    t = row_up_i<2>(seg); if (c16 >= 2) seg += t;
    t = row_up_i<4>(seg); if (c16 >= 4) seg += t;
    t = row_up_i<8>(seg); if (c16 >= 8) seg += t;
    const int s1 = row_down_i<1>(seg), s2 = row_down_i<2>(seg), s4 = row_down_i<4>(seg), s8 = row_down_i<8>(seg);
    run.take1 = (c16 + 1 < 16) & (s1 == seg);
    run.take2 = (c16 + 2 < 16) & (s2 == seg);
    run.take4 = (c16 + 4 < 16) & (s4 == seg);
    run.take8 = (c16 + 8 < 16) & (s8 == seg);
}

template <int F>
__device__ __forceinline__ void dx_from_entries(const LevelInfo& L, const Cell& c, const float g[F], const float tv[8][F], float dx[3]) {
    float dot[8];
#pragma unroll
    for (int k = 0; k < 8; ++k) {
        dot[k] = 0.0f;
#pragma unroll
        for (int f = 0; f < F; ++f) dot[k] += g[f] * tv[k][f];
    }
    const float fx = c.frac[0], fy = c.frac[1], fz = c.frac[2];
    const float gx = 1.0f - fx, gy = 1.0f - fy, gz = 1.0f - fz;
    const float dxv = ((dot[1] - dot[0]) * gy + (dot[3] - dot[2]) * fy) * gz + ((dot[5] - dot[4]) * gy + (dot[7] - dot[6]) * fy) * fz;
    const float dyv = ((dot[2] - dot[0]) * gx + (dot[3] - dot[1]) * fx) * gz + ((dot[6] - dot[4]) * gx + (dot[7] - dot[5]) * fx) * fz;
    const float dzv = ((dot[4] - dot[0]) * gx + (dot[5] - dot[1]) * fx) * gy + ((dot[6] - dot[2]) * gx + (dot[7] - dot[3]) * fx) * fy;
    dx[0] = dxv * L.scale; dx[1] = dyv * L.scale; dx[2] = dzv * L.scale;
}

#define ENC_DX_NONE 0
#define ENC_DX_PLANES 1
#define ENC_DX_RAYS 2

__device__ __forceinline__ float row_sum_all(float v) {
    v += __int_as_float(__builtin_amdgcn_update_dpp(0, __float_as_int(v), 0xB1, 0xF, 0xF, true));
    v += __int_as_float(__builtin_amdgcn_update_dpp(0, __float_as_int(v), 0x4E, 0xF, 0xF, true));
    v += __int_as_float(__builtin_amdgcn_update_dpp(0, __float_as_int(v), 0x141, 0xF, 0xF, true));
    v += __int_as_float(__builtin_amdgcn_update_dpp(0, __float_as_int(v), 0x140, 0xF, 0xF, true));
    return v;
}
__device__ __forceinline__ float rows_sum_all(float v) {
    typedef unsigned u2 __attribute__((ext_vector_type(2)));
    const unsigned a = __float_as_uint(v);
    const u2 r = __builtin_amdgcn_permlane16_swap(a, a, false, false);
    const float s = __uint_as_float(r.x) + __uint_as_float(r.y);
    const unsigned b = __float_as_uint(s);
    const u2 q = __builtin_amdgcn_permlane32_swap(b, b, false, false);
    return __uint_as_float(q.x) + __uint_as_float(q.y);
}
__device__ __forceinline__ void ray_accumulate_dx(float* __restrict__ ray_acc_f, uint32_t ray, float z, const float dx[3], int lane, int n_rays_cap) {
    long long* ray_acc = reinterpret_cast<long long*>(ray_acc_f);
    const int c16 = lane & 15;
    float v = row_sum_all(dx[0]);
    { const float t = row_sum_all(dx[1]); if (c16 == 1) v = t; }
    { const float t = row_sum_all(dx[2]); if (c16 == 2) v = t; }
    { const float t = row_sum_all(z * dx[0]); if (c16 == 3) v = t; }
    { const float t = row_sum_all(z * dx[1]); if (c16 == 4) v = t; }
    { const float t = row_sum_all(z * dx[2]); if (c16 == 5) v = t; }
    v = rows_sum_all(v);
    if (lane < 6) {
        if (__builtin_expect(__builtin_isfinite(v), 1)) {
            if (v != 0.0f) atomicAdd(reinterpret_cast<unsigned long long*>(ray_acc) + (size_t)ray * 6 + lane,
                                     (unsigned long long)__float2ll_rn(0.5f * v * LNR_FIX_SCALE));
        } else {
            ray_acc[(size_t)n_rays_cap * 6 + ray] = 1ll;
        }
    }
}

__global__ void __launch_bounds__(ENC_BLOCK)
ray_grad_apply_kernel(const long long* __restrict__ ray_acc, int n_rays, const int32_t* __restrict__ n_rays_dev, float* __restrict__ d_rays) {
    const int i = blockIdx.x * ENC_BLOCK + threadIdx.x;
    if (i >= lnr_live_rays(n_rays, n_rays_dev) * 6) return;
    const long long q = ray_acc[i];
    if (__builtin_expect(ray_acc[(size_t)n_rays * 6 + i / 6] != 0ll, 0)) d_rays[(size_t)(i / 6) * LNR_RAY_STRIDE + (i % 6)] = __builtin_nanf("");
    else if (q != 0ll) d_rays[(size_t)(i / 6) * LNR_RAY_STRIDE + (i % 6)] += (float)((double)q * (1.0 / (double)LNR_FIX_SCALE));
}

__device__ __forceinline__ void store_stream_b128(uint64_t global_addr, uint4 v) {
    typedef uint32_t u32x4 __attribute__((ext_vector_type(4)));
    const u32x4 q = {v.x, v.y, v.z, v.w};
    asm volatile("global_store_dwordx4 %0, %1, off nt" :: "v"(global_addr), "v"(q) : "memory");
}

#define ENC_BWD_BLOCK LNR_ENC_BWD_BLOCK
#define ENC_STAGE_RECORDS (ENC_BWD_BLOCK * 8)

struct OwnerSlot {
    uint32_t ptr_lo, ptr_hi;
    int scan;
    int room;
};

__device__ __forceinline__ void xpair_overflow(long long* ovf_level, uint32_t fi0_in_level, uint32_t fi1_in_level, uint32_t t, float a0, float a1, float fx) {
    uint32_t pi, tt; float q0, q1, qx;
    lnr_unpack_xpair(lnr_pack_xpair(0u, t, a0, a1, fx), pi, tt, q0, q1, qx);
    long long q[4];
    lnr_xpair_fix(q0, q1, qx, q);
    unsigned long long* o = reinterpret_cast<unsigned long long*>(ovf_level);
    atomicAdd(o + fi0_in_level, (unsigned long long)q[0]);
    atomicAdd(o + fi0_in_level + 1, (unsigned long long)q[1]);
    atomicAdd(o + fi1_in_level, (unsigned long long)q[2]);
    atomicAdd(o + fi1_in_level + 1, (unsigned long long)q[3]);
}

#ifdef LNR_PHASE_TIMING
__device__ unsigned long long lnr_phase_cycles[2 * LNR_N_PHASES];
#endif

template <int F, int DXM, bool XP>
#ifndef LNR_ENC_BWD_WAVES
#define LNR_ENC_BWD_WAVES 4
#endif
__global__ void __launch_bounds__(ENC_BWD_BLOCK, LNR_ENC_BWD_WAVES)
encode_backward_kernel(const LnrNetSpec spec, const float* __restrict__ table, const PointSrc src, const float* __restrict__ dfeat,
                       float* __restrict__ dxl, int64_t m_pad, int bpg, const LevelList list, const EncSink sink) {
    constexpr bool WANT_DX = DXM != ENC_DX_NONE;
    extern __shared__ __attribute__((aligned(16))) int dyn[];
    __shared__ int s_total;
    constexpr bool PAIR = F >= 2;
    constexpr int NPASS = PAIR ? F / 2 : 1;
    const int maxo = sink.maxo;
    const int maxo4 = (maxo + 3) & ~3;
    int* cnt = dyn;
    int* gcur = dyn + maxo4;
    OwnerSlot* oslot = reinterpret_cast<OwnerSlot*>(dyn + 2 * maxo4);
    void* stage = reinterpret_cast<void*>(dyn + 2 * maxo4 + 4 * maxo);
    for (int i = threadIdx.x; i < maxo; i += ENC_BWD_BLOCK) { cnt[i] = 0; gcur[i] = 0; }
    __syncthreads();
    int slot, chunk;
    if (!level_slot(bpg, list.n, sink.xcd_affine != 0, slot, chunk)) return;
    const int lv = list.lv[slot];
    const LevelInfo L = level_info(spec, lv);
    const int lane = threadIdx.x & 63, wave = threadIdx.x >> 6;
    const uint32_t M = (uint32_t)live_points(src);
    const int first_owner = (int)(((uint64_t)L.offset * F) >> sink.shift);
    constexpr bool xp = XP && F == 2;
    const bool combine = !xp && L.scale < sink.combine_scale_max;
    const uint32_t rec_bytes = xp ? 12u : 8u;
    const uint32_t region_bytes = sink.plan.bytes[lv];
    const int cap_rec = (int)(region_bytes / rec_bytes);
    const char* level_regions = reinterpret_cast<const char*>(sink.regions) + sink.plan.off[lv];
    const int ovf_off = list.slab_off[slot];
    long long* ovf = ovf_off >= 0 ? sink.ovf + ovf_off : nullptr;
    const uint32_t level_base = L.offset * F;
    const size_t region0 = (size_t)lv * maxo * bpg + chunk;
    const size_t region_step = (size_t)bpg;
    const uint32_t step = (uint32_t)bpg * ENC_BWD_BLOCK;
    const uint32_t n_iter = (M + step - 1u) / step;
    const float* gplanes = dfeat + (size_t)(lv * F) * m_pad;
    float* dxplanes = dxl + (size_t)(lv * 3) * m_pad;
    const uint32_t plane_bytes = (uint32_t)m_pad * 4u;
    const bool emit = sink.regions != nullptr;
    if (M == 0u) {
        if (emit) for (int i = threadIdx.x; i < maxo; i += ENC_BWD_BLOCK) sink.counts[region0 + i * region_step] = 0;
        return;
    }

    constexpr bool EARLY_DX = WANT_DX && F <= 2;
    SampleCursor cur;
    cur.init((uint32_t)chunk * ENC_BWD_BLOCK + threadIdx.x, step, src.pts ? 1u : (uint32_t)src.n_samples);
    const uint32_t last_ray = src.pts ? 0u : (M - 1u) / cur.S;
    const bool uni = ray_uniform(src, 64u);
    float g_next[F];
    RawPoint p_next;
    {
        const bool in = cur.m < M;
        const uint32_t mc = in ? cur.m : M - 1u;
#pragma unroll
        for (int f = 0; f < F; ++f) g_next[f] = ld32_stream<float>(gplanes, (uint32_t)f * plane_bytes + mc * 4u);
        load_raw_point(src, mc, in ? cur.ray : last_ray, p_next, uni);
    }
    PHASE_INIT();
    for (uint32_t it = 0; it < n_iter; ++it) {
        PHASE(11);
        const uint32_t m = cur.m;
        const bool live = m < M;
        float g[F];
        bool any = false;
#pragma unroll
        for (int f = 0; f < F; ++f) { g[f] = live ? g_next[f] : 0.0f; any |= (g[f] != 0.0f); }
        const RawPoint p_cur = p_next;
        const uint32_t ray_cur = cur.ray;
        cur.advance();
        {
            const bool in = cur.m < M;
            const uint32_t mc = in ? cur.m : M - 1u;
#pragma unroll
            for (int f = 0; f < F; ++f) g_next[f] = ld32_stream<float>(gplanes, (uint32_t)f * plane_bytes + mc * 4u);
            load_raw_point(src, mc, in ? cur.ray : last_ray, p_next, uni);
        }
        const bool wave_any = __ballot(any) != 0ull;
        PHASE(0);
        Cell c;
        uint32_t e[8];
        float w[8];
        bool head = true;
        RunMask run = {false, false, false, false};
        float tv[EARLY_DX ? 8 : 1][F];
        if (wave_any) {
            float x[3];
            unit_point(src, p_cur, x);
            c = cell_of(L, x);
            cell_entries(L, c, e);
            if constexpr (EARLY_DX) { if (any) gather_entries<F>(table, e, tv); }
            cell_weights(c, w);
            if (combine) cell_runs(c, lane, head, run);
        }
        PHASE(1);
#pragma unroll
        for (int pass = 0; pass < (emit ? NPASS : 0); ++pass) {
            float rv0[8], rv1[8]; int rrank[8];
#pragma unroll
            for (int k = 0; k < 8; ++k) rrank[k] = -1;
            uint32_t xt = 0u;
            if (wave_any && xp) {
                xt = (uint32_t)__builtin_ctz(~c.b[0]);
                const float wy[2] = {1.0f - c.frac[1], c.frac[1]}, wz[2] = {1.0f - c.frac[2], c.frac[2]};
#pragma unroll
                for (int k2 = 0; k2 < 4; ++k2) {
                    const float wyz = wy[k2 & 1] * wz[k2 >> 1];
                    const float a0 = wyz * g[0], a1 = wyz * g[F >= 2 ? 1 : 0];
                    rv0[k2] = a0; rv1[k2] = a1;
                    if ((a0 != 0.0f) | (a1 != 0.0f)) {
                        const uint32_t fi = e[2 * k2] * F;
                        if (xt < 12u) rrank[k2] = atomicAdd(&cnt[(int)(fi >> sink.shift) - first_owner], 1);
                        else {
                            const uint32_t fj = e[2 * k2 + 1] * F;
                            const float gx = 1.0f - c.frac[0];
// ... 384 lines not shown
                                            (uint32_t)__builtin_amdgcn_readlane((int)gpos, ((j0 + j) * BPI + 1) * G);
                        if (half) dst = d1;
                    }
                    if ((uint32_t)piece < n16[j]) store_stream_b128(dst + (uint32_t)piece * 16u, v[j]);
                }
            }
            if (mv) {
                uint4 t4[TQ];
#pragma unroll
                for (int q = 0; q < TQ; ++q) if (sub + 16u * q < rem) t4[q] = *reinterpret_cast<const uint4*>(my_bin + (nlines << 7) + sub + 16u * q);
#pragma unroll
                for (int q = 0; q < TQ; ++q) if (sub + 16u * q < rem) *reinterpret_cast<uint4*>(my_bin + sub + 16u * q) = t4[q];
            }
            gpos += nlines << 7;
            tail = rem;
            if (!closed && gpos + (uint32_t)(BIN + 128) > region_bytes) {
                char* dst = level_regions + ((size_t)my_owner * bpg + chunk) * (size_t)region_bytes + gpos;
#pragma unroll
                for (int q = 0; q < 32 / G; ++q) {
                    const uint32_t off = sub + 4u * q;
                    if (off < rem) *reinterpret_cast<uint32_t*>(dst + off) = *reinterpret_cast<const uint32_t*>(my_bin + off);
                }
                gpos += rem;
                tail = 0u;
                closed = true;
            }
            if (lane % G == 0 && own) fill[my_owner] = closed ? ENC_BIN_CLOSED : (int)tail;
            __syncthreads();
        }
        if constexpr (WANT_DX) {
            float dx[3] = {0.0f, 0.0f, 0.0f};
            if (any) {
                if constexpr (EARLY_DX) dx_from_entries<F>(L, c, g, tv, dx);
                else { float tl[8][F]; gather_entries<F>(table, e, tl); dx_from_entries<F>(L, c, g, tl, dx); }
            }
            if constexpr (DXM == ENC_DX_RAYS) {
                if (wave_any) ray_accumulate_dx(dxl, (uint32_t)__builtin_amdgcn_readfirstlane((int)ray_cur), p_cur.z, dx, lane, src.n_rays);
            } else if (live) {
#pragma unroll
                for (int d = 0; d < 3; ++d) st32<float>(dxplanes, (uint32_t)d * plane_bytes + m * 4u, dx[d]);
            }
        }
    }
    if (emit && own) {
        if (!closed && tail > 0u) {
            const char* my_bin = stage + (uint32_t)my_owner * BIN;
            char* dst = level_regions + ((size_t)my_owner * bpg + chunk) * (size_t)region_bytes + gpos;
            const uint32_t sub = (uint32_t)(lane % G) * (128u / G);
#pragma unroll
            for (int q = 0; q < 32 / G; ++q) {
                const uint32_t off = sub + 4u * q;
                if (off < tail) *reinterpret_cast<uint32_t*>(dst + off) = *reinterpret_cast<const uint32_t*>(my_bin + off);
            }
        }
        if (lane % G == 0) sink.counts[region0 + (size_t)my_owner * region_step] = (int)((gpos + (closed ? 0u : tail)) / REC);
    }
}

__global__ void __launch_bounds__(ENC_BLOCK)
freq_backward_kernel(const LnrNetSpec spec, const PointSrc src, const float* __restrict__ dfeat, float* __restrict__ dxl, int64_t m_pad) {
    const int64_t M = live_points(src);
    const int nf = spec.n_frequencies;
    for (int64_t m = (int64_t)blockIdx.x * ENC_BLOCK + threadIdx.x; m < M; m += (int64_t)gridDim.x * ENC_BLOCK) {
        float x[3];
        load_unit_point(src, m, x);
        float dx[3];
#pragma unroll
        for (int dim = 0; dim < 3; ++dim) {
            float acc = 0.0f;
            for (int f = 0; f < nf; ++f) {
                const uint32_t k = (uint32_t)(2 * (dim * nf + f));
                const float d0 = dfeat[(size_t)k * (size_t)m_pad + (size_t)m], d1 = dfeat[(size_t)(k + 1u) * (size_t)m_pad + (size_t)m];
                const float mult = __uint_as_float((uint32_t)(127 + f) << 23);
                const float ph = lnr_mul_rn(lnr_mul_rn(x[dim], mult), LNR_PI_F);
                float sn, cs;
                sincos_f32(ph, &sn, &cs);
                const float h = lnr_add_rn(ph, LNR_PI_2_F);
                const float bb = lnr_add_rn(h, -ph);
                const float e = lnr_add_rn(lnr_add_rn(ph, -lnr_add_rn(h, -bb)), lnr_add_rn(LNR_PI_2_F, -bb));
                const float dl = 4.371139000186243e-8f - e;
                acc += (d0 * cs - d1 * __builtin_fmaf(dl, cs, sn)) * (mult * LNR_PI_F);
            }
            dx[dim] = acc;
        }
#pragma unroll
        for (int d = 0; d < 3; ++d) dxl[(size_t)d * m_pad + m] = dx[d];
    }
}

__global__ void __launch_bounds__(ENC_BLOCK)
sum_dx_planes_kernel(const float* __restrict__ dxl, int n_groups, int64_t m_pad, const PointSrc src, float* __restrict__ d_pts) {
    const int64_t M = live_points(src);
    for (int64_t m = (int64_t)blockIdx.x * ENC_BLOCK + threadIdx.x; m < M; m += (int64_t)gridDim.x * ENC_BLOCK) {
        float a[3] = {0.0f, 0.0f, 0.0f};
        for (int gI = 0; gI < n_groups; ++gI) {
#pragma unroll
            for (int d = 0; d < 3; ++d) a[d] += dxl[(size_t)(gI * 3 + d) * m_pad + m];
        }
        d_pts[3 * m] = 0.5f * a[0]; d_pts[3 * m + 1] = 0.5f * a[1]; d_pts[3 * m + 2] = 0.5f * a[2];
    }
}

int lnr_encode_forward(const LnrNetSpec* spec, const float* params, const PointSrc* src, int64_t cap_points, float* feat,
                       int64_t m_pad, bool half_planes, hipStream_t st) {
    const float* table = params + spec->n_mlp_params;
    const bool hash = spec->encoding == LNR_ENC_HASHGRID;
    const int n_groups = hash ? spec->n_levels : (spec->enc_dim + 3) / 4;
    int64_t bpg = (cap_points + ENC_BLOCK * 4 - 1) / (ENC_BLOCK * 4);
    if (bpg < 1) bpg = 1;
    if (bpg > 2048) bpg = 2048;
    const dim3 grid((unsigned)(n_groups * bpg)), block(ENC_BLOCK);
    if (!hash) {
        if (half_planes) {
            int64_t b1 = (cap_points + ENC_BLOCK - 1) / ENC_BLOCK;
            if (b1 < 1) b1 = 1;
            if (b1 > 16384) b1 = 16384;
            hipLaunchKernelGGL(freq_forward_h16_kernel, dim3((unsigned)(3 * b1)), block, 0, st, *spec, *src, reinterpret_cast<uint32_t*>(feat), m_pad, (int)b1);
        } else {
            hipLaunchKernelGGL(freq_forward_kernel, grid, block, 0, st, *spec, *src, feat, m_pad, (int)bpg);
        }
        return LNR_OK;
    }
    const uint32_t level_mask = spec->n_levels >= 32 ? 0xFFFFFFFFu : (1u << spec->n_levels) - 1u;
    const dim3 mgrid((unsigned)(__builtin_popcount(level_mask) * bpg));
    const int xcd = lnr_xcd_affine(__builtin_popcount(level_mask), cap_points, true) ? 1 : 0;
#define LNR_FWD(F, H) hipLaunchKernelGGL((encode_forward_kernel<F, H>), mgrid, block, 0, st, *spec, table, *src, feat, m_pad, (int)bpg, level_mask, xcd)
    if (half_planes) {
        switch (spec->n_features) {
            case 2: LNR_FWD(2, true); break;
            case 4: LNR_FWD(4, true); break;
            case 8: LNR_FWD(8, true); break;
            default: lnr_set_error("fp16 feature planes pair up features: n_features_per_level must be even"); return LNR_ERR_UNSUPPORTED;
        }
    } else {
        switch (spec->n_features) {
            case 1: LNR_FWD(1, false); break;
            case 2: LNR_FWD(2, false); break;
            case 4: LNR_FWD(4, false); break;
            default: LNR_FWD(8, false); break;
        }
    }
#undef LNR_FWD
    return LNR_OK;
}

int lnr_encode_backward(const LnrNetSpec* spec, const float* params, const PointSrc* src, int64_t cap_points, const float* dfeat,
                        float* dxl, int64_t m_pad, float* grad_table, void* regions, const RegionPlan* plan, int* counts, int bpg,
                        int maxo, int shift, long long* ovf, int* ovf_flag, int epoch, float* d_pts, float* d_rays_acc, long long* ray_acc, bool bins_w8,
                        hipStream_t st) {
    const float* table = params + spec->n_mlp_params;
    const bool hash = spec->encoding == LNR_ENC_HASHGRID;
    const int dxm = d_rays_acc ? ENC_DX_RAYS : (d_pts ? ENC_DX_PLANES : ENC_DX_NONE);
    float* dx_out = d_rays_acc ? reinterpret_cast<float*>(ray_acc) : dxl;
    if (d_rays_acc && hipMemsetAsync(ray_acc, 0, ((((size_t)src->n_rays * 7) * sizeof(long long)) + 15) & ~(size_t)15, st) != hipSuccess) {
        lnr_set_error("lnr_density_backward: hipMemsetAsync failed");
        return LNR_ERR_LAUNCH;
    }
    int n_groups = 1;
    if (hash) n_groups = spec->n_levels;
    if (hash && (regions != nullptr || dxm != ENC_DX_NONE)) {
        LevelList rec_levels, xp_levels, brec_levels, bxp_levels;
        rec_levels.n = xp_levels.n = brec_levels.n = bxp_levels.n = 0;
        const bool allow_binned = regions != nullptr && maxo <= LNR_BIN_MAX_OWNERS;
        int ovf_total = 0;
        for (int l = 0; l < spec->n_levels; ++l) {
            const int nfl = (int)spec->level_size[l] * spec->n_features;
            const bool is_xp = spec->n_features == 2 && plan->xp[l] != 0;
            const bool is_binned = allow_binned && plan->binned[l] != 0 && plan->bytes[l] != 0;
            LevelList& ll = is_xp ? (is_binned ? bxp_levels : xp_levels) : (is_binned ? brec_levels : rec_levels);
            ll.lv[ll.n] = l; ll.slab_off[ll.n] = ovf_total; ll.n++;
            ovf_total += nfl;
        }
        const dim3 block(ENC_BWD_BLOCK);
#define LNR_LAUNCH_DXM(KERNEL, F, XP, ...)                                                                                    \
        do {                                                                                                                  \
            hipError_t e_ = hipSuccess;                                                                                       \
            const void* fn_ = dxm == ENC_DX_RAYS ? reinterpret_cast<const void*>(KERNEL<F, ENC_DX_RAYS, XP>)                  \
                            : dxm == ENC_DX_PLANES ? reinterpret_cast<const void*>(KERNEL<F, ENC_DX_PLANES, XP>)              \
                                                   : reinterpret_cast<const void*>(KERNEL<F, ENC_DX_NONE, XP>);               \
            e_ = hipFuncSetAttribute(fn_, hipFuncAttributeMaxDynamicSharedMemorySize, (int)lds);                              \
            if (e_ != hipSuccess) { lnr_set_error("lnr_density_backward: hipFuncSetAttribute(%zu) failed", lds); return LNR_ERR_LAUNCH; } \
            if (dxm == ENC_DX_RAYS) hipLaunchKernelGGL((KERNEL<F, ENC_DX_RAYS, XP>), grid, block, lds, st, __VA_ARGS__);   \
            else if (dxm == ENC_DX_PLANES) hipLaunchKernelGGL((KERNEL<F, ENC_DX_PLANES, XP>), grid, block, lds, st, __VA_ARGS__); \
            else hipLaunchKernelGGL((KERNEL<F, ENC_DX_NONE, XP>), grid, block, lds, st, __VA_ARGS__);                      \
        } while (0)
#define LNR_LAUNCH_F(KERNEL, ...)                                                   \
        switch (spec->n_features) {                                                 \
            case 1: LNR_LAUNCH_DXM(KERNEL, 1, false, __VA_ARGS__); break;           \
            case 2: LNR_LAUNCH_DXM(KERNEL, 2, false, __VA_ARGS__); break;           \
            case 4: LNR_LAUNCH_DXM(KERNEL, 4, false, __VA_ARGS__); break;           \
            default: LNR_LAUNCH_DXM(KERNEL, 8, false, __VA_ARGS__); break;          \
        }
        if (rec_levels.n + xp_levels.n + brec_levels.n + bxp_levels.n > 0) {
            EncSink sink;
            sink.ovf_flag = ovf_flag; sink.epoch = epoch;
            sink.grad_table = grad_table; sink.ovf = ovf; sink.regions = regions; sink.plan = *plan; sink.counts = counts; sink.maxo = maxo; sink.shift = shift;
            sink.combine_scale_max = LNR_COMBINE_SCALE_MAX;
            LnrProfScope prof("encode_backward", st);
            const int maxo4 = (maxo + 3) & ~3;
            const size_t lds = (size_t)(2 * maxo4 + 4 * maxo) * sizeof(int) + (size_t)ENC_STAGE_RECORDS * (spec->n_features >= 2 ? 16 : 8);
            if (rec_levels.n > 0) {
                const dim3 grid((unsigned)(rec_levels.n * bpg));
                sink.xcd_affine = lnr_xcd_affine(rec_levels.n, cap_points, false) ? 1 : 0;
                LNR_LAUNCH_F(encode_backward_kernel, *spec, table, *src, dfeat, dx_out, m_pad, bpg, rec_levels, sink);
            }
            if (xp_levels.n > 0) {
                const dim3 grid((unsigned)(xp_levels.n * bpg));
                sink.xcd_affine = lnr_xcd_affine(xp_levels.n, cap_points, false) ? 1 : 0;
                LNR_LAUNCH_DXM(encode_backward_kernel, 2, true, *spec, table, *src, dfeat, dx_out, m_pad, bpg, xp_levels, sink);
            }
            {
                const int nw = bins_w8 ? 8 : 4;
                const size_t lds_b = 64 * sizeof(int) + (size_t)LNR_BIN_MAX_OWNERS * (size_t)(128 * nw);
                const dim3 block_b(64 * nw);
#define LNR_LAUNCH_BINNED(F, XP, LIST)                                                                                              \
                do {                                                                                                                \
                    const dim3 grid_b((unsigned)((LIST).n * bpg));                                                                  \
                    sink.xcd_affine = lnr_xcd_affine((LIST).n, cap_points, false) ? 1 : 0;                                                             \
                    const void* fn_ = nullptr;                                                                                      \
                    if (nw == 8) fn_ = dxm == ENC_DX_RAYS ? (const void*)encode_backward_binned_kernel<F, ENC_DX_RAYS, XP, 8>       \
                                     : dxm == ENC_DX_PLANES ? (const void*)encode_backward_binned_kernel<F, ENC_DX_PLANES, XP, 8>   \
                                                            : (const void*)encode_backward_binned_kernel<F, ENC_DX_NONE, XP, 8>;    \
                    else fn_ = dxm == ENC_DX_RAYS ? (const void*)encode_backward_binned_kernel<F, ENC_DX_RAYS, XP, 4>               \
                             : dxm == ENC_DX_PLANES ? (const void*)encode_backward_binned_kernel<F, ENC_DX_PLANES, XP, 4>           \
                                                    : (const void*)encode_backward_binned_kernel<F, ENC_DX_NONE, XP, 4>;            \
                    if (hipFuncSetAttribute(fn_, hipFuncAttributeMaxDynamicSharedMemorySize, (int)lds_b) != hipSuccess) {           \
                        lnr_set_error("lnr_density_backward: hipFuncSetAttribute(%zu) failed", lds_b); return LNR_ERR_LAUNCH;       \
                    }                                                                                                               \
                    void* args_[] = {(void*)spec, (void*)&table, (void*)src, (void*)&dfeat, (void*)&dx_out, (void*)&m_pad, (void*)&bpg, (void*)&(LIST), (void*)&sink}; \
                    if (hipLaunchKernel(fn_, grid_b, block_b, args_, lds_b, st) != hipSuccess) {                                    \
                        lnr_set_error("lnr_density_backward: launch of the binned partition failed"); return LNR_ERR_LAUNCH;         \
                    }                                                                                                               \
                } while (0)
                if (brec_levels.n > 0) {
                    switch (spec->n_features) {
                        case 2: LNR_LAUNCH_BINNED(2, false, brec_levels); break;
                        case 4: LNR_LAUNCH_BINNED(4, false, brec_levels); break;
                        default: LNR_LAUNCH_BINNED(8, false, brec_levels); break;
                    }
                }
                if (bxp_levels.n > 0) LNR_LAUNCH_BINNED(2, true, bxp_levels);
#undef LNR_LAUNCH_BINNED
            }
#ifdef LNR_PHASE_TIMING
            if (getenv("LNR_PHASE_TIMING")) {
                static const char* names[LNR_N_PHASES] = {"load inputs", "cell/entries/gather/weights", "A rank", "barrier 1", "B scan", "barrier 2",
                                                          "C stage", "barrier 3", "D copy-out", "dx", "-", "loop"};
                unsigned long long h[2 * LNR_N_PHASES];
                if (lnr_phase_fetch(HIP_SYMBOL(lnr_phase_cycles), h, 2 * LNR_N_PHASES, st)) {
                    lnr_phase_print("encode_backward 8-byte", names, h);
                    lnr_phase_print("encode_backward x-pair", names, h + LNR_N_PHASES);
                }
            }
#endif
        }
#undef LNR_LAUNCH_F
#undef LNR_LAUNCH_DXM
    } else if (!hash && dxm != ENC_DX_NONE) {
        int64_t blocks = (cap_points + ENC_BLOCK - 1) / ENC_BLOCK;
        if (blocks > 4096) blocks = 4096;
        hipLaunchKernelGGL(freq_backward_kernel, dim3((unsigned)blocks), dim3(ENC_BLOCK), 0, st, *spec, *src, dfeat, dxl, m_pad);
    }
    if (dxm == ENC_DX_RAYS) {
        hipLaunchKernelGGL(ray_grad_apply_kernel, dim3((unsigned)((src->n_rays * 6 + ENC_BLOCK - 1) / ENC_BLOCK)), dim3(ENC_BLOCK), 0, st,
                           ray_acc, src->n_rays, src->n_rays_dev, d_rays_acc);
    }
    if (dxm == ENC_DX_PLANES) {
        int64_t blocks = (cap_points + ENC_BLOCK - 1) / ENC_BLOCK;
        if (blocks > 4096) blocks = 4096;
        LnrProfScope prof("sum_dx_planes", st);
        hipLaunchKernelGGL(sum_dx_planes_kernel, dim3((unsigned)blocks), dim3(ENC_BLOCK), 0, st, dxl, n_groups, m_pad, *src, d_pts);
    }
    return LNR_OK;
}
```

loner_amd/csrc/lnr_render.hip:

```cpp
#include "lnr_common.h"
#include "lnr_render_ray.h"

__device__ __forceinline__ float wave_excl_suffix_sum(float v, int lane) {
    float inc = v;
#pragma unroll
    for (int o = 1; o < 64; o <<= 1) {
        float t = __shfl_down(inc, o, 64);
        if (lane + o < 64) inc += t;
    }
    float ex = __shfl_down(inc, 1, 64);
    return lane == 63 ? 0.0f : ex;
}

template <int C>
__device__ __forceinline__ void render_ray_backward(const RayState<C>& st, const float G[C], float g_far, int ray, int S, int lane,
                                                    const float* __restrict__ rayrec, float* __restrict__ d_sigma,
                                                    float* __restrict__ d_rays) {
    const int base = lane * C;
    float gw[C];
    float local = 0.0f;
#pragma unroll
    for (int t = 0; t < C; ++t) { gw[t] = G[t] * st.w[t]; local += gw[t]; }
    const float behind_lanes = wave_excl_suffix_sum(local, lane);
    float suffix = behind_lanes;
// ... 41 lines not shown
    if (lane == 0) {
        if (depth) depth[ray] = st.depth;
        if (opacity) opacity[ray] = st.opacity;
        if (variance) variance[ray] = st.variance;
    }
}

template <int C>
__global__ void __launch_bounds__(RENDER_BLOCK)
render_backward_kernel(const float* __restrict__ sigma, const float* __restrict__ z, const float* __restrict__ rays, int n_rays,
                       const int32_t* __restrict__ n_rays_dev, int S, const float* __restrict__ noise, float noise_std,
                       uint64_t seed, const float* __restrict__ g_depth, const float* __restrict__ g_weights,
                       const float* __restrict__ g_opacity, const float* __restrict__ g_variance,
                       float* __restrict__ d_sigma, float* __restrict__ d_rays) {
    const int lane = threadIdx.x & 63;
    const int ray = blockIdx.x * RAYS_PER_BLOCK + (threadIdx.x >> 6);
    if (ray >= lnr_live_rays(n_rays, n_rays_dev)) return;
    const float* rr = rays + (size_t)ray * LNR_RAY_STRIDE;
    RayState<C> st;
    render_ray<C>(st, sigma, z, noise, noise_std, seed, ray, S, lane, rr);
    const float gD = g_depth ? g_depth[ray] : 0.0f;
    const float gO = g_opacity ? g_opacity[ray] : 0.0f;
    const float gV = g_variance ? g_variance[ray] : 0.0f;
    float q_part = 0.0f;
#pragma unroll
    for (int t = 0; t < C; ++t) q_part += st.w[t] * (st.depth - st.z[t]);
    const float gD_tot = gD + gV * 2.0f * wave_sum(q_part);
    const float far = rr[12];
    float G[C];
#pragma unroll
    for (int t = 0; t < C; ++t) {
        const int i = lane * C + t;
        const float q = st.depth - st.z[t];
        float g = gO + gD_tot * (st.z[t] - far) + gV * q * q;
        if (g_weights && i < S) g += g_weights[(size_t)ray * S + i];
        G[t] = (i < S) ? g : 0.0f;
    }
    render_ray_backward<C>(st, G, gD_tot * (1.0f - st.opacity), ray, S, lane, rr, d_sigma, d_rays);
}

__device__ __forceinline__ float std_normal_cdf(float x) { return 0.5f * (1.0f + erff(x / 1.41421356237309515f)); }

__device__ __forceinline__ float target_raw(float s, float g, float eps, float sd, float clip_norm) {
    const bool inside = (s - (g - eps) > 0.0f) && ((g + eps) - s > 0.0f);
    if (!inside) return 0.0f;
    const float t = (s - g) / sd;
    return 0.39894228040143270f * expf(-0.5f * (t * t)) / sd / clip_norm;
}

__device__ __forceinline__ void target_params(float g, float eps, float* sd, float* clip_norm) {
    *sd = eps / 3.0f;
    const float lo = (g - eps - g) / *sd;
    const float hi = (g + eps - g) / *sd;
    *clip_norm = std_normal_cdf(hi) - std_normal_cdf(lo);
}

__device__ __forceinline__ float gaussian_kl(float m1, float s1, float m2, float s2) {
    const float d = m1 - m2;
    return logf(s2 / s1) + (s1 * s1 + d * d) / (2.0f * (s2 * s2)) - 0.5f;
}
__device__ __forceinline__ float gaussian_js(float m1, float s1, float m2, float s2) {
    const float mm = 0.5f * (m1 + m2);
    const float sm = 0.5f * sqrtf(s1 * s1 + s2 * s2);
    return 0.5f * gaussian_kl(m1, s1, mm, sm) + 0.5f * gaussian_kl(m2, s2, mm, sm);
}

template <int C>
__device__ __forceinline__ void los_loss_ray(const float* __restrict__ sigma, const float* __restrict__ z, const float* __restrict__ rays,
                                             const float* __restrict__ depth_gt, int S, const float* __restrict__ noise, float noise_std,
                                             uint64_t seed, float scale, const LnrLossConfig& cfg, const int32_t* __restrict__ counts,
                                             float* terms, bool terms_atomic, float* __restrict__ d_sigma, float* __restrict__ d_rays,
                                             float* __restrict__ ray_stats, float* __restrict__ weights_out, int ray, int lane,
                                             const float* __restrict__ far0_dev) {
    const float* rr = rays + (size_t)ray * LNR_RAY_STRIDE;
    RayState<C> st;
    render_ray<C>(st, sigma, z, noise, noise_std, seed, ray, S, lane, rr);

    const float dgt = depth_gt[ray];
    const float far0 = far0_dev ? far0_dev[0] : rays[12];
    const bool opaque = (dgt > 0.0f) && !(dgt > far0);
    const float g = dgt * scale;
    const float n_all = (float)counts[0] * (float)S;
    const float n_op = (float)counts[1];

    float m_part = 0.0f;
#pragma unroll
    for (int t = 0; t < C; ++t) m_part += (st.z[t] * scale) * st.w[t];
    const float wden = st.opacity + 1e-10f;
    const float mean = wave_sum(m_part) / wden;
    float v_part = 0.0f;
#pragma unroll
    for (int t = 0; t < C; ++t) { const float q = st.z[t] * scale - mean; v_part += q * q * st.w[t]; }
    const float var = wave_sum(v_part) / wden + 1e-10f;
    const float sd_pred = sqrtf(var);
    const float js = gaussian_js(g, cfg.min_eps / 3.0f, mean, sd_pred);

    float eps;
    if (cfg.selection <= 1) {
        float score = js;
        if (score < cfg.min_js) score = 0.0f;
        if (score > cfg.max_js) score = cfg.max_js;
        eps = cfg.min_eps * (1.0f + cfg.js_alpha * score);
    } else {
        eps = cfg.fixed_eps;
    }
    float sd_t, clip_norm;
    target_params(g, eps, &sd_t, &clip_norm);
    float raw[C];
    float r_part = 0.0f;
#pragma unroll
    for (int t = 0; t < C; ++t) {
        raw[t] = (lane * C + t < S) ? target_raw(st.z[t] * scale, g, eps, sd_t, clip_norm) : 0.0f;
        r_part += raw[t];
    }
    const float rden = wave_sum(r_part) + 1e-6f;

    const bool l1 = (cfg.selection == 0 || cfg.selection == 2);
    const float depth_m = st.depth * scale;
    const float gO = opaque ? ((st.opacity - 1.0f > 0.0f) ? 1.0f : (st.opacity - 1.0f < 0.0f ? -1.0f : 0.0f)) / n_op : 0.0f;
    const float gD = opaque ? cfg.depth_lambda * 2.0f * (depth_m - g) * scale / n_op : 0.0f;
    const float far = rr[12];
    float G[C];
    float los_part = 0.0f;
#pragma unroll
    for (int t = 0; t < C; ++t) {
        const int i = lane * C + t;
        const float target = opaque ? raw[t] / rden : 0.0f;
        const float diff = st.w[t] - target;
        float gw;
        if (l1) { los_part += fabsf(diff); gw = (diff > 0.0f ? 1.0f : (diff < 0.0f ? -1.0f : 0.0f)); }
        else { los_part += diff * diff; gw = 2.0f * diff; }
        G[t] = (i < S) ? cfg.los_lambda * gw / n_all + gO + gD * (st.z[t] - far) : 0.0f;
        if (weights_out && i < S) weights_out[(size_t)ray * S + i] = st.w[t];
    }
    const float los_sum = wave_sum(los_part);
    render_ray_backward<C>(st, G, gD * (1.0f - st.opacity), ray, S, lane, rr, d_sigma, d_rays);

    if (lane == 0) {
        const float l_depth = opaque ? cfg.depth_lambda * (depth_m - g) * (depth_m - g) / n_op : 0.0f;
        const float l_los = cfg.los_lambda * los_sum / n_all;
        const float l_op = opaque ? fabsf(st.opacity - 1.0f) / n_op : 0.0f;
        const float t5[5] = {l_depth + l_los + l_op, l_depth, l_los, l_op, eps};
#pragma unroll
        for (int q = 0; q < 5; ++q) { if (terms_atomic) atomicAdd(terms + q, t5[q]); else terms[q] = t5[q]; }
        if (ray_stats) {
            float* o = ray_stats + (size_t)ray * 8;
            o[0] = st.depth; o[1] = st.opacity; o[2] = st.variance; o[3] = mean; o[4] = sd_pred; o[5] = js; o[6] = eps;
            o[7] = opaque ? 1.0f : 0.0f;
        }
    }
}


template <int C>
__global__ void __launch_bounds__(RENDER_BLOCK)
los_loss_fused_kernel(const float* __restrict__ sigma, const float* __restrict__ z, const float* __restrict__ rays,
                      const float* __restrict__ depth_gt, int n_rays, const int32_t* __restrict__ n_rays_dev, int S,
                      const float* __restrict__ noise, float noise_std, uint64_t seed, float scale, const LnrLossConfig cfg,
                      const int32_t* __restrict__ counts, float* __restrict__ loss_out, float* __restrict__ d_sigma,
                      float* __restrict__ d_rays, float* __restrict__ ray_stats, float* __restrict__ weights_out,
                      float* __restrict__ block_partials, const float* __restrict__ far0_dev) {
    __shared__ float s_terms[RAYS_PER_BLOCK][5];
    const int lane = threadIdx.x & 63;
    const int ray = blockIdx.x * RAYS_PER_BLOCK + (threadIdx.x >> 6);
    const bool alive = ray < lnr_live_rays(n_rays, n_rays_dev);
    if (block_partials) {
        if (lane < 5) s_terms[threadIdx.x >> 6][lane] = 0.0f;
        if (alive) los_loss_ray<C>(sigma, z, rays, depth_gt, S, noise, noise_std, seed, scale, cfg, counts, s_terms[threadIdx.x >> 6], false,
                                   d_sigma, d_rays, ray_stats, weights_out, ray, lane, far0_dev);
        __syncthreads();
        if (threadIdx.x < 8) {
            float v = 0.0f;
            if (threadIdx.x < 5) for (int r = 0; r < RAYS_PER_BLOCK; ++r) v += s_terms[r][threadIdx.x];
            block_partials[(size_t)blockIdx.x * 8 + threadIdx.x] = v;
        }
    } else if (alive) {
        los_loss_ray<C>(sigma, z, rays, depth_gt, S, noise, noise_std, seed, scale, cfg, counts, loss_out, true,
                        d_sigma, d_rays, ray_stats, weights_out, ray, lane, far0_dev);
    }
}

__global__ void loss_reduce_kernel(const float* __restrict__ block_partials, int n_blocks, float* __restrict__ loss_out,
                                   int32_t* __restrict__ poison, int32_t poison_tag) {
    __shared__ float part[4][8];
    const int term = threadIdx.x & 7, slice = threadIdx.x >> 3;
    float v = 0.0f;
    for (int b = slice; b < n_blocks; b += 32) v += block_partials[(size_t)b * 8 + term];
    v += __shfl_xor(v, 8, 64); v += __shfl_xor(v, 16, 64); v += __shfl_xor(v, 32, 64);
    if ((threadIdx.x & 63) < 8) part[threadIdx.x >> 6][term] = v;
    __syncthreads();
    if (threadIdx.x < 5) {
        const float t = loss_out[threadIdx.x] + (part[0][threadIdx.x] + part[1][threadIdx.x] + part[2][threadIdx.x] + part[3][threadIdx.x]);
        loss_out[threadIdx.x] = t;
        if (threadIdx.x == 0 && poison != nullptr && t != t && atomicCAS(poison, 0, LNR_POISON_NAN_LOSS) == 0) poison[1] = poison_tag;
    }
}

__global__ void count_opaque_kernel(const float* __restrict__ rays, const float* __restrict__ depth_gt, int n_rays,
                                    const int32_t* __restrict__ n_rays_dev, int32_t* __restrict__ counts,
                                    const float* __restrict__ far0_dev) {
    __shared__ int partial[16];
    const int n = lnr_live_rays(n_rays, n_rays_dev);
    const float far0 = far0_dev ? far0_dev[0] : (n > 0 ? rays[12] : 0.0f);
    int c = 0;
    for (int i = threadIdx.x; i < n; i += blockDim.x) {
        const float d = depth_gt[i];
        c += ((d > 0.0f) && !(d > far0)) ? 1 : 0;
    }
    for (int o = 32; o > 0; o >>= 1) c += __shfl_xor(c, o, 64);
    if ((threadIdx.x & 63) == 0) partial[threadIdx.x >> 6] = c;
    __syncthreads();
    if (threadIdx.x == 0) {
        int t = 0;
        for (int w = 0; w < (int)(blockDim.x >> 6); ++w) t += partial[w];
        counts[0] = n;
        counts[1] = t;
    }
}

__global__ void weights_gt_kernel(const float* __restrict__ s, const float* __restrict__ g, const float* __restrict__ eps_ray,
                                  float eps_scalar, int normalise, int n_rays, int S, float* __restrict__ out) {
    const int lane = threadIdx.x & 63;
    const int ray = blockIdx.x * RAYS_PER_BLOCK + (threadIdx.x >> 6);
    if (ray >= n_rays) return;
    const float gg = g[ray];
    const float eps = eps_ray ? eps_ray[ray] : eps_scalar;
    float sd, cn;
    target_params(gg, eps, &sd, &cn);
    float part = 0.0f;
    for (int i = lane; i < S; i += 64) part += target_raw(s[(size_t)ray * S + i], gg, eps, sd, cn);
    const float den = wave_sum(part) + 1e-6f;
    for (int i = lane; i < S; i += 64) {
        const float v = target_raw(s[(size_t)ray * S + i], gg, eps, sd, cn);
        out[(size_t)ray * S + i] = normalise ? v / den : v;
    }
}

__global__ void logits_grad_kernel(const float* __restrict__ s, const float* __restrict__ g, int64_t total, int S, float margin,
                                   float l_free, float l_occ, float* __restrict__ out) {
    const int64_t i = (int64_t)blockIdx.x * blockDim.x + threadIdx.x;
    if (i >= total) return;
    const float x = s[i] - g[i / S];
    const float free_side = (-x - margin > 0.0f) ? 1.0f : 0.0f;
    const float near_surface = ((x + margin > 0.0f) && (margin - x > 0.0f)) ? 1.0f : 0.0f;
    out[i] = l_free * free_side - l_occ * near_surface;
}

__global__ void points_grad_to_rays_kernel(const float* __restrict__ d_pts, const float* __restrict__ z, int n_rays,
                                           const int32_t* __restrict__ n_rays_dev, int S, float* __restrict__ d_rays) {
    const int lane = threadIdx.x & 63;
    const int ray = blockIdx.x * RAYS_PER_BLOCK + (threadIdx.x >> 6);
    if (ray >= lnr_live_rays(n_rays, n_rays_dev)) return;
    float a[6] = {0.0f, 0.0f, 0.0f, 0.0f, 0.0f, 0.0f};
    for (int i = lane; i < S; i += 64) {
        const size_t m = (size_t)ray * S + i;
        const float zv = z[m];
        const float gx = d_pts[3 * m], gy = d_pts[3 * m + 1], gz = d_pts[3 * m + 2];
        a[0] += gx; a[1] += gy; a[2] += gz;
        a[3] += zv * gx; a[4] += zv * gy; a[5] += zv * gz;
    }
#pragma unroll
    for (int k = 0; k < 6; ++k) a[k] = wave_sum(a[k]);
    if (lane < 6) {
        float v = lane == 0 ? a[0] : lane == 1 ? a[1] : lane == 2 ? a[2] : lane == 3 ? a[3] : lane == 4 ? a[4] : a[5];
        d_rays[(size_t)ray * LNR_RAY_STRIDE + lane] += v;
    }
}


extern "C" int lnr_render_forward(const float* sigma, const float* z, const float* rays, int32_t n_rays, const int32_t* n_rays_dev,
                                  int32_t n_samples, const float* noise, float noise_std, uint64_t seed, float* depth,
                                  float* weights, float* opacity, float* variance, void* stream) {
    LNR_REQUIRE(sigma && z && rays && n_rays >= 0 && n_samples >= 2, "lnr_render_forward: bad argument");
    if (n_rays == 0) return LNR_OK;
    const dim3 grid(lnr_div_up(n_rays, RAYS_PER_BLOCK)), block(RENDER_BLOCK);
    hipStream_t st = (hipStream_t)stream;
    DISPATCH_C(n_samples, hipLaunchKernelGGL(render_forward_kernel<C>, grid, block, C >= 16 ? RAYS_PER_BLOCK * 64 * (C + 4) * sizeof(float) : 0, st,
                                             sigma, z, rays, n_rays, n_rays_dev, n_samples, noise, noise_std, seed, depth, weights, opacity, variance));
    LNR_CHECK_LAUNCH("lnr_render_forward");
    return LNR_OK;
}

#define FTB_T_MIN 5.9604644775390625e-08f

__global__ void __launch_bounds__(RENDER_BLOCK)
ftb_gather_kernel(const float* __restrict__ rays, const float* __restrict__ z, int S, const int32_t* __restrict__ idx,
                  const int32_t* __restrict__ n_alive, int cap, int b0, int B, float* __restrict__ rays_c, float* __restrict__ z_c,
                  int32_t* __restrict__ next_count) {
    if (blockIdx.x == 0 && threadIdx.x == 0) *next_count = 0;
    const int lane = threadIdx.x & 63;
    const int n = min(*n_alive, cap);
    for (int j = blockIdx.x * RAYS_PER_BLOCK + (threadIdx.x >> 6); j < n; j += gridDim.x * RAYS_PER_BLOCK) {
        const int ray = idx[j];
        if (lane < LNR_RAY_STRIDE) rays_c[(size_t)j * LNR_RAY_STRIDE + lane] = rays[(size_t)ray * LNR_RAY_STRIDE + lane];
        const float* src = z + (size_t)ray * S + b0;
        float* dst = z_c + (size_t)j * B;
        for (int i = 4 * lane; i < B; i += 256) *reinterpret_cast<float4*>(dst + i) = *reinterpret_cast<const float4*>(src + i);
    }
}

__global__ void __launch_bounds__(RENDER_BLOCK)
ftb_composite_kernel(const float* __restrict__ sigma_c, const float* __restrict__ z, const float* __restrict__ rays, int S,
                     const int32_t* __restrict__ idx, const int32_t* __restrict__ n_alive, int cap, int b0, const float* __restrict__ noise,
                     float noise_std, uint64_t seed, float* __restrict__ T_ray, float* __restrict__ depth_acc, float* __restrict__ opac_acc,
                     int32_t* __restrict__ next_idx, int32_t* __restrict__ next_count, int last) {
    constexpr int C = 4, B = 64 * C;
    const int lane = threadIdx.x & 63;
    const int n = min(*n_alive, cap);
    for (int j = blockIdx.x * RAYS_PER_BLOCK + (threadIdx.x >> 6); j < n; j += gridDim.x * RAYS_PER_BLOCK) {
        const int ray = idx[j];
        const float* rec = rays + (size_t)ray * LNR_RAY_STRIDE;
        const float dnorm = sqrtf(rec[3] * rec[3] + rec[4] * rec[4] + rec[5] * rec[5]);
        const int i0 = b0 + C * lane;
        const float4 zv = *reinterpret_cast<const float4*>(z + (size_t)ray * S + i0);
        const float4 sv = *reinterpret_cast<const float4*>(sigma_c + (size_t)j * B + C * lane);
        const float zl[C] = {zv.x, zv.y, zv.z, zv.w};
        float dens[C] = {sv.x, sv.y, sv.z, sv.w};
        if (noise != nullptr) {
            const float4 nv = *reinterpret_cast<const float4*>(noise + (size_t)ray * S + i0);
            dens[0] += nv.x; dens[1] += nv.y; dens[2] += nv.z; dens[3] += nv.w;
        } else if (noise_std > 0.0f) {
#pragma unroll
            for (int t = 0; t < C; ++t) dens[t] += lnr_rand_normal(seed, (uint64_t)ray, (uint32_t)(i0 + t)) * noise_std;
        }
        float z_after = __shfl_down(zl[0], 1, 64);
        if (lane == 63) z_after = (b0 + B < S) ? z[(size_t)ray * S + b0 + B] : 0.0f;
        float e[C], Tl[C], tprod = 1.0f;
#pragma unroll
        for (int t = 0; t < C; ++t) {
            const int i = i0 + t;
            float delta = (i < S - 1) ? ((t + 1 < C) ? zl[(t + 1 < C) ? t + 1 : t] : z_after) - zl[t] : 1e10f;
            delta *= dnorm;
            const float r = dens[t] > 0.0f ? dens[t] : 0.0f;
            e[t] = expf(-delta * r);
            Tl[t] = tprod;
            tprod *= (1.0f - (1.0f - e[t]) + 1e-10f);
        }
        const float prefix = wave_excl_prod(tprod, lane) * T_ray[ray];
        float o_part = 0.0f, d_part = 0.0f;
#pragma unroll
        for (int t = 0; t < C; ++t) {
            const float w = (1.0f - e[t]) * (Tl[t] * prefix);
            o_part += w;
            d_part += w * zl[t];
        }
        const float o_sum = wave_sum(o_part), d_sum = wave_sum(d_part);
        const float T_out = __shfl(prefix * tprod, 63, 64);
        if (lane == 0) {
            depth_acc[ray] += d_sum;
            opac_acc[ray] += o_sum;
            T_ray[ray] = T_out;
            if (!last && T_out >= FTB_T_MIN) next_idx[atomicAdd(next_count, 1)] = ray;
        }
    }
}

extern "C" int lnr_render_ftb_gather(const float* rays, const float* z, int32_t n_samples, const int32_t* idx, const int32_t* n_alive_dev,
                                     int32_t cap, int32_t b0, int32_t block_samples, float* rays_c, float* z_c, int32_t* next_count_dev,
                                     void* stream) {
    LNR_REQUIRE(rays && z && idx && n_alive_dev && rays_c && z_c && next_count_dev, "lnr_render_ftb_gather: null argument");
    LNR_REQUIRE(cap >= 0 && block_samples > 0 && block_samples % 4 == 0 && b0 >= 0 && b0 % 4 == 0 && b0 + block_samples <= n_samples && n_samples % 4 == 0,
                "lnr_render_ftb_gather: a block must lie inside the ray's samples (multiples of four)");
    if (cap == 0) return LNR_OK;
    const int blocks = lnr_div_up(cap, RAYS_PER_BLOCK);
    hipLaunchKernelGGL(ftb_gather_kernel, dim3(blocks > 4096 ? 4096 : blocks), dim3(RENDER_BLOCK), 0, (hipStream_t)stream, rays, z, n_samples, idx,
                       n_alive_dev, cap, b0, block_samples, rays_c, z_c, next_count_dev);
    LNR_CHECK_LAUNCH("lnr_render_ftb_gather");
    return LNR_OK;
}

extern "C" int lnr_render_ftb_composite(const float* sigma_c, const float* z, const float* rays, int32_t n_samples, const int32_t* idx,
                                        const int32_t* n_alive_dev, int32_t cap, int32_t b0, int32_t block_samples, const float* noise, float noise_std,
                                        uint64_t seed, float* transmittance, float* depth_acc, float* opacity_acc, int32_t* next_idx, int32_t* next_count_dev,
                                        int32_t last, void* stream) {
    LNR_REQUIRE(sigma_c && z && rays && idx && n_alive_dev && transmittance && depth_acc && opacity_acc && next_idx && next_count_dev,
                "lnr_render_ftb_composite: null argument");
    LNR_REQUIRE(block_samples == 256, "lnr_render_ftb_composite: blocks of 256 samples (one wave per ray, four samples per lane)");
    LNR_REQUIRE(cap >= 0 && b0 >= 0 && b0 % 4 == 0 && b0 + block_samples <= n_samples && n_samples % 4 == 0, "lnr_render_ftb_composite: a block must lie inside the ray's samples");
    if (cap == 0) return LNR_OK;
    const int blocks = lnr_div_up(cap, RAYS_PER_BLOCK);
    hipLaunchKernelGGL(ftb_composite_kernel, dim3(blocks > 4096 ? 4096 : blocks), dim3(RENDER_BLOCK), 0, (hipStream_t)stream, sigma_c, z, rays, n_samples,
                       idx, n_alive_dev, cap, b0, noise, noise_std, seed, transmittance, depth_acc, opacity_acc, next_idx, next_count_dev, last);
    LNR_CHECK_LAUNCH("lnr_render_ftb_composite");
    return LNR_OK;
}

extern "C" int lnr_render_backward(const float* sigma, const float* z, const float* rays, int32_t n_rays, const int32_t* n_rays_dev,
                                   int32_t n_samples, const float* noise, float noise_std, uint64_t seed, const float* g_depth,
                                   const float* g_weights, const float* g_opacity, const float* g_variance, float* d_sigma,
                                   float* d_rays, void* stream) {
    LNR_REQUIRE(sigma && z && rays && d_sigma && d_rays && n_rays >= 0 && n_samples >= 2, "lnr_render_backward: bad argument");
    if (n_rays == 0) return LNR_OK;
    const dim3 grid(lnr_div_up(n_rays, RAYS_PER_BLOCK)), block(RENDER_BLOCK);
    hipStream_t st = (hipStream_t)stream;
    DISPATCH_C(n_samples, hipLaunchKernelGGL(render_backward_kernel<C>, grid, block, 0, st, sigma, z, rays, n_rays, n_rays_dev, n_samples,
                                             noise, noise_std, seed, g_depth, g_weights, g_opacity, g_variance, d_sigma, d_rays));
    LNR_CHECK_LAUNCH("lnr_render_backward");
    return LNR_OK;
}

extern "C" int lnr_count_opaque(const float* rays, const float* depth_gt, int32_t n_rays, const int32_t* n_rays_dev,
                                const float* far0_dev, int32_t* counts_dev, void* stream) {
    LNR_REQUIRE(counts_dev && n_rays >= 0 && (n_rays == 0 || (rays && depth_gt)), "lnr_count_opaque: bad argument");
    hipLaunchKernelGGL(count_opaque_kernel, dim3(1), dim3(1024), 0, (hipStream_t)stream, rays, depth_gt, n_rays, n_rays_dev, counts_dev,
                       far0_dev);
    LNR_CHECK_LAUNCH("lnr_count_opaque");
    return LNR_OK;
}

extern "C" int lnr_los_loss_fused(const float* sigma, const float* z, const float* rays, const float* depth_gt, int32_t n_rays,
                                  const int32_t* n_rays_dev, int32_t n_samples, const float* noise, float noise_std, uint64_t seed,
                                  float scale, const LnrLossConfig* cfg, const int32_t* counts_dev, const float* far0_dev, float* loss_out,
                                  float* d_sigma, float* d_rays, float* ray_stats, float* weights_out, float* block_partials,
                                  int32_t* poison_dev, int32_t poison_tag, void* stream) {
    LNR_REQUIRE(sigma && z && rays && depth_gt && cfg && counts_dev && loss_out && d_sigma && d_rays, "lnr_los_loss_fused: null argument");
    LNR_REQUIRE(poison_dev == nullptr || block_partials != nullptr, "lnr_los_loss_fused: the failure guard needs block_partials (the deterministic reduction)");
    LNR_REQUIRE(cfg->selection >= 0 && cfg->selection <= 3, "lnr_los_loss_fused: unknown loss selection %d", cfg->selection);
    LNR_REQUIRE(n_rays >= 0 && n_samples >= 2, "lnr_los_loss_fused: bad sizes");
    if (n_rays == 0) return LNR_OK;
    const dim3 grid(lnr_div_up(n_rays, RAYS_PER_BLOCK)), block(RENDER_BLOCK);
    hipStream_t st = (hipStream_t)stream;
    DISPATCH_C(n_samples, hipLaunchKernelGGL(los_loss_fused_kernel<C>, grid, block, 0, st, sigma, z, rays, depth_gt, n_rays, n_rays_dev,
                                             n_samples, noise, noise_std, seed, scale, *cfg, counts_dev, loss_out, d_sigma, d_rays,
                                             ray_stats, weights_out, block_partials, far0_dev));
    LNR_CHECK_LAUNCH("lnr_los_loss_fused");
    if (block_partials) {
        hipLaunchKernelGGL(loss_reduce_kernel, dim3(1), dim3(256), 0, st, block_partials, (int)grid.x, loss_out, poison_dev, poison_tag);
        LNR_CHECK_LAUNCH("lnr_los_loss_fused(reduce)");
    }
    return LNR_OK;
}

extern "C" int lnr_weights_gt(const float* s, const float* g, const float* eps_ray, float eps_scalar, int32_t normalise,
                              int32_t n_rays, int32_t n_samples, float* out, void* stream) {
    LNR_REQUIRE(s && g && out && n_rays >= 0 && n_samples > 0, "lnr_weights_gt: bad argument");
    if (n_rays == 0) return LNR_OK;
    hipLaunchKernelGGL(weights_gt_kernel, dim3(lnr_div_up(n_rays, RAYS_PER_BLOCK)), dim3(RENDER_BLOCK), 0, (hipStream_t)stream, s, g,
                       eps_ray, eps_scalar, normalise, n_rays, n_samples, out);
    LNR_CHECK_LAUNCH("lnr_weights_gt");
    return LNR_OK;
}

extern "C" int lnr_logits_grad(const float* s, const float* g, int32_t n_rays, int32_t n_samples, float margin, float l_free,
                               float l_occ, float* out, void* stream) {
    LNR_REQUIRE(s && g && out && n_rays >= 0 && n_samples > 0, "lnr_logits_grad: bad argument");
    const int64_t total = (int64_t)n_rays * n_samples;
    if (total == 0) return LNR_OK;
    hipLaunchKernelGGL(logits_grad_kernel, dim3(lnr_div_up(total, 256)), dim3(256), 0, (hipStream_t)stream, s, g, total, n_samples,
                       margin, l_free, l_occ, out);
    LNR_CHECK_LAUNCH("lnr_logits_grad");
    return LNR_OK;
}

extern "C" int lnr_points_grad_to_rays(const float* d_pts, const float* z, int32_t n_rays, const int32_t* n_rays_dev,
                                       int32_t n_samples, float* d_rays, void* stream) {
    LNR_REQUIRE(d_pts && z && d_rays && n_rays >= 0 && n_samples > 0, "lnr_points_grad_to_rays: bad argument");
    if (n_rays == 0) return LNR_OK;
    hipLaunchKernelGGL(points_grad_to_rays_kernel, dim3(lnr_div_up(n_rays, RAYS_PER_BLOCK)), dim3(RENDER_BLOCK), 0, (hipStream_t)stream,
                       d_pts, z, n_rays, n_rays_dev, n_samples, d_rays);
    LNR_CHECK_LAUNCH("lnr_points_grad_to_rays");
    return LNR_OK;
}


__global__ void noise_draws_kernel(uint64_t seed, int n_rays, int n_per_ray, float* __restrict__ out) {
    const int64_t i = (int64_t)blockIdx.x * blockDim.x + threadIdx.x;
    if (i >= (int64_t)n_rays * n_per_ray) return;
    out[i] = lnr_rand_normal(seed, (uint64_t)(i / n_per_ray), (uint32_t)(i % n_per_ray));
}

int lnr_render_noise_draws(uint64_t seed, int n_rays, int n_per_ray, float* out, hipStream_t st) {
    const int64_t n = (int64_t)n_rays * n_per_ray;
    hipLaunchKernelGGL(noise_draws_kernel, dim3((unsigned)((n + 255) / 256)), dim3(256), 0, st, seed, n_rays, n_per_ray, out);
    LNR_CHECK_LAUNCH("lnr_rng_draws");
    return LNR_OK;
}
```

loner_amd/ops.py:

```python
import ctypes as C
import math
import os

import torch

from . import hip
from .hip import _ptr, _stream, check, load, require_device

_steps_cache = {}


def linspace_table(count: int, device) -> torch.Tensor:
    key = (count, str(device))
    t = _steps_cache.get(key)
    if t is None:
        t = torch.linspace(0, 1, count).to(device)
        _steps_cache[key] = t
    return t


def _f32c(t):
    if t is None:
        return None
    if t.dtype != torch.float32:
# ... 515 lines not shown
        check(lib.lnr_nn_grid_build(_ptr(pts), self.n, edge, _ptr(ws), need, _ptr(self.buf), gbytes, _ptr(info), _stream()),
              "lnr_nn_grid_build")
        info = info.cpu()
        _cloud_status("NNGrid", info)
        self.n_cells = int(info[1])
        self.edge = float(info[4:5].view(torch.float64)[0])
        self.dims = tuple(int(x) for x in info[5:8])

    def distance(self, queries, want_sq=False, stats=None):
        q = _f64_points(queries, "NNGrid.distance")
        m = q.shape[0]
        dev = q.device
        dist = torch.empty(m, device=dev, dtype=torch.float64)
        d2 = torch.empty(m, device=dev, dtype=torch.float64) if want_sq else None
        ws, need = _cloud_workspace(m, dev)
        counters = torch.empty(4, device=dev, dtype=torch.int64)
        check(load().lnr_nn_distance(_ptr(self.buf), self.n, _ptr(q), m, _ptr(dist), _ptr(d2), _ptr(ws), need, _ptr(counters),
                                     _stream()), "lnr_nn_distance")
        c = counters.cpu()
        if int(c[1]):
            raise RuntimeError(f"compute_point_cloud_distance: {int(c[1])} queries with non-finite coordinates")
        if stats is not None:
            stats.update(fallback=int(c[0]), shells=int(c[2]))
        return (dist, d2) if want_sq else dist

    def normals(self, knn=30, want_covariances=False, stats=None):
        knn = int(knn)
        if not 1 <= knn <= hip.KNN_MAX:
            raise ValueError(f"normals: knn must be in [1, {hip.KNN_MAX}], got {knn}")
        dev = self.buf.device
        normals = torch.empty(self.n, 3, device=dev, dtype=torch.float64)
        cov = torch.empty(self.n, 3, 3, device=dev, dtype=torch.float64) if want_covariances else None
        ws, need = _cloud_workspace(self.n, dev)
        counters = torch.empty(4, device=dev, dtype=torch.int64)
        check(load().lnr_cloud_normals(_ptr(self.buf), self.n, knn, _ptr(normals), _ptr(cov), _ptr(ws), need, _ptr(counters), _stream()),
              "lnr_cloud_normals")
        c = counters.cpu()
        if int(c[1]):
            raise RuntimeError("normals: the grid is unusable (non-finite targets)")
        if stats is not None:
            stats.update(fallback=int(c[0]), shells=int(c[2]))
        return (normals, cov) if want_covariances else normals

    def correspondences(self, queries, max_distance):
        q = _f64_points(queries, "NNGrid.correspondences")
        r = float(max_distance)
        if not (math.isfinite(r) and r > 0):
            raise ValueError(f"correspondences: max_distance must be finite and > 0, got {max_distance!r}")
        m = q.shape[0]
        index = torch.empty(m, device=q.device, dtype=torch.int32)
        d2 = torch.empty(m, device=q.device, dtype=torch.float64)
        counters = torch.empty(4, device=q.device, dtype=torch.int64)
        check(load().lnr_icp_correspondences(_ptr(self.buf), self.n, _ptr(q), m, r, _ptr(index), _ptr(d2), _ptr(counters), _stream()),
              "lnr_icp_correspondences")
        if int(counters[1].item()):
            raise RuntimeError(f"correspondences: {int(counters[1].item())} queries with non-finite coordinates")
        return index, d2


_ICP_STATUS = {1: "non-finite source points", 2: "the target grid is unusable (non-finite targets)", 4: "non-finite target normals",
               8: "the update is not finite (a degenerate system)"}


def icp_point_to_plane(grid, target_normals, source, max_distance, init=None, relative_fitness=1e-6, relative_rmse=1e-6,
                       max_iteration=30):
    import numpy as np
    src = _f64_points(source, "icp_point_to_plane")
    nrm = _f64_points(target_normals, "icp_point_to_plane")
    if nrm.shape[0] != grid.n:
        raise ValueError(f"icp_point_to_plane: {nrm.shape[0]} normals for {grid.n} targets")
    r = float(max_distance)
    if not (math.isfinite(r) and r > 0):
        raise ValueError(f"icp_point_to_plane: max_correspondence_distance must be finite and > 0, got {max_distance!r}")
    T0 = np.eye(4) if init is None else np.asarray(init.detach().cpu().numpy() if torch.is_tensor(init) else init, dtype=np.float64)
    if T0.shape != (4, 4) or not np.array_equal(T0[3], [0.0, 0.0, 0.0, 1.0]) or not np.isfinite(T0).all():
        raise ValueError(f"icp_point_to_plane: init must be a finite 4x4 affine matrix, got {T0.tolist()}")
    dev = src.device
    lib = load()
    need = int(lib.lnr_icp_workspace(src.shape[0]))
    ws = torch.empty(need, device=dev, dtype=torch.uint8)
    result = torch.empty(hip.ICP_RESULT, device=dev, dtype=torch.float64)
    info = torch.empty(8, device=dev, dtype=torch.int64)
    t16 = (C.c_double * 16)(*[float(x) for x in T0.reshape(-1)])
    check(lib.lnr_icp_point_to_plane(_ptr(grid.buf), grid.n, _ptr(nrm), _ptr(src), src.shape[0], r, t16, float(relative_fitness),
                                     float(relative_rmse), int(max_iteration), _ptr(ws), need, _ptr(result), _ptr(info), _stream()),
          "lnr_icp_point_to_plane")
    res = result.cpu().numpy()
    info = [int(x) for x in info.cpu()]
    if info[0]:
        raise RuntimeError("icp_point_to_plane: " + ", ".join(m for b, m in _ICP_STATUS.items() if info[0] & b))
    JTJ = np.zeros((6, 6))
    JTJ[np.triu_indices(6)] = res[18:39]
    JTJ = JTJ + np.triu(JTJ, 1).T
    return {"transformation": res[:16].reshape(4, 4).copy(), "fitness": float(res[16]), "inlier_rmse": float(res[17]),
            "n_correspondences": info[1], "iterations": info[2], "JTJ": JTJ, "JTr": res[39:45].copy(), "sum_d2": float(res[45]),
            "x": res[46:52].copy(), "system_correspondences": info[5]}


def render_backward(sigma, z, rays, g_depth, g_weights, g_opacity, g_variance, noise=None, noise_std=0.0, seed=0,
                    n_rays_dev=None):
    require_device(sigma, z, rays)
    sigma, z, rays = _f32c(sigma), _f32c(z), _f32c(rays)
    n, s = z.shape
    d_sigma = torch.zeros(n, s, device=z.device)
    d_rays = torch.zeros(n, hip.RAY_STRIDE, device=z.device)
    check(load().lnr_render_backward(_ptr(sigma), _ptr(z), _ptr(rays), n, _ptr(n_rays_dev), s, _ptr(_f32c(noise)),
                                     float(noise_std), int(seed), _ptr(_f32c(g_depth)), _ptr(_f32c(g_weights)),
                                     _ptr(_f32c(g_opacity)), _ptr(_f32c(g_variance)), _ptr(d_sigma), _ptr(d_rays), _stream()),
          "lnr_render_backward")
    return d_sigma, d_rays


def points_grad_to_rays(d_pts, z, d_rays, n_rays_dev=None):
    require_device(d_pts, z, d_rays)
    n, s = z.shape
    check(load().lnr_points_grad_to_rays(_ptr(_f32c(d_pts)), _ptr(_f32c(z)), n, _ptr(n_rays_dev), s, _ptr(d_rays), _stream()),
          "lnr_points_grad_to_rays")
    return d_rays


def weights_gt(s, g, eps, normalise=True):
    require_device(s, g)
    s = _f32c(s)
    n, k = s.shape
    g = _f32c(g).reshape(-1)
    out = torch.empty_like(s)
    if isinstance(eps, torch.Tensor):
        require_device(eps)
        e = _f32c(eps).reshape(-1)
        check(load().lnr_weights_gt(_ptr(s), _ptr(g), _ptr(e), 0.0, int(normalise), n, k, _ptr(out), _stream()), "lnr_weights_gt")
    else:
        check(load().lnr_weights_gt(_ptr(s), _ptr(g), None, float(eps), int(normalise), n, k, _ptr(out), _stream()), "lnr_weights_gt")
    return out


def logits_grad(s, g, margin=2.0, l_free=0.25, l_occ=2.5):
    require_device(s, g)
    s = _f32c(s)
    n, k = s.shape
    out = torch.empty_like(s)
    check(load().lnr_logits_grad(_ptr(s), _ptr(_f32c(g).reshape(-1)), n, k, float(margin), float(l_free), float(l_occ),
                                 _ptr(out), _stream()), "lnr_logits_grad")
    return out


def count_opaque(rays, depth_gt, n_rays_dev=None, far0=None):
    require_device(rays, depth_gt, far0)
    counts = torch.empty(2, device=rays.device, dtype=torch.int32)
    check(load().lnr_count_opaque(_ptr(_f32c(rays)), _ptr(_f32c(depth_gt)), rays.shape[0], _ptr(n_rays_dev), _ptr(far0),
                                  _ptr(counts), _stream()), "lnr_count_opaque")
    return counts


def los_loss_fused(sigma, z, rays, depth_gt, scale, cfg: hip.LossConfig, counts, noise=None, noise_std=0.0, seed=0,
                   n_rays_dev=None, want_stats=False, want_weights=False, loss_out=None, far0=None, poison=None, poison_tag=0,
                   zero_dead_rows=True):
    require_device(sigma, z, rays, depth_gt, counts, noise, far0, poison)
    sigma, z, rays, depth_gt = _f32c(sigma), _f32c(z), _f32c(rays), _f32c(depth_gt)
    n, s = z.shape
    dev = z.device
    if loss_out is None:
        loss_out = torch.zeros(8, device=dev)
    d_sigma = torch.empty(n, s, device=dev)
    d_rays = (torch.zeros if (zero_dead_rows and n_rays_dev is not None) else torch.empty)(n, hip.RAY_STRIDE, device=dev)
    stats = torch.zeros(n, 8, device=dev) if want_stats else None
    w = torch.zeros(n, s, device=dev) if want_weights else None
    partials = torch.empty(((n + hip.LOSS_RAYS_PER_BLOCK - 1) // hip.LOSS_RAYS_PER_BLOCK) * 8, device=dev)
    check(load().lnr_los_loss_fused(_ptr(sigma), _ptr(z), _ptr(rays), _ptr(depth_gt), n, _ptr(n_rays_dev), s,
                                    _ptr(_f32c(noise)), float(noise_std), int(seed), float(scale), C.byref(cfg), _ptr(counts),
                                    _ptr(far0), _ptr(loss_out), _ptr(d_sigma), _ptr(d_rays), _ptr(stats), _ptr(w), _ptr(partials),
                                    _ptr(poison), int(poison_tag), _stream()),
          "lnr_los_loss_fused")
    return loss_out, d_sigma, d_rays, stats, w


def adam_step(params, grads, exp_avg, exp_avg_sq, lr, step, betas=(0.9, 0.999), eps=1e-8, grad_scale=1.0, zero_grad=True, poison=None):
    require_device(params, grads, exp_avg, exp_avg_sq, poison)
    check(load().lnr_adam_step(_ptr(params), _ptr(grads), _ptr(exp_avg), _ptr(exp_avg_sq), params.numel(), float(lr),
                               float(betas[0]), float(betas[1]), float(eps), int(step), float(grad_scale), int(zero_grad),
                               _ptr(poison), _stream()), "lnr_adam_step")


def occ_grid_step(grid, rays, z, depth_gt, scale, lr, margin=2.0, l_free=0.25, l_occ=2.5, grad_buf=None, n_rays_dev=None):
    require_device(grid, rays, z, depth_gt, grad_buf)
    assert grad_buf is None or (grad_buf.dtype == torch.int64 and grad_buf.is_contiguous())
    v = grid.shape[-1]
    n, s = z.shape
    check(load().lnr_occ_grid_step(_ptr(grid), v, _ptr(_f32c(rays)), _ptr(_f32c(z)), _ptr(_f32c(depth_gt)), n, _ptr(n_rays_dev),
                                   s, float(scale), float(lr), float(margin), float(l_free), float(l_occ), _ptr(grad_buf),
                                   _stream()), "lnr_occ_grid_step")


def occ_grid_apply(grid, grad_buf, lr, zero_grad=True, poison=None):
    require_device(grid, grad_buf, poison)
    assert grad_buf.dtype == torch.int64 and grad_buf.is_contiguous()
    check(load().lnr_occ_grid_apply(_ptr(grid), _ptr(grad_buf), grid.numel(), float(lr), int(zero_grad), _ptr(poison), _stream()),
          "lnr_occ_grid_apply")


def rng_draws(which, seed, n_rays, n_per_ray, device="cuda"):
    out = torch.empty(int(n_rays), int(n_per_ray), device=device, dtype=torch.float32)
    check(load().lnr_rng_draws(int(which), int(seed) & (2 ** 64 - 1), int(n_rays), int(n_per_ray), _ptr(out), _stream()), "lnr_rng_draws")
    return out


def selftest_mfma(device="cuda"):
    out = torch.full((3,), -1.0, device=device)
    check(load().lnr_selftest_mfma(_ptr(out), _stream()), "lnr_selftest_mfma")
    return float(out.abs().max().item()) if bool((out >= 0).all()) else -1.0
```

Measured before the change: 2.037 million.

## Fuse loss reduce, restructure bf3 backward LDS tiles, skip empty reduce blocks

Several independent changes. The separate loss reduce kernel is folded into the loss kernel using a last-block ticket over a persistent partials buffer. The ray-accumulator memset is skipped when a workspace is known to be already zero. Table-grad reduce blocks exit early when all their region counts are zero. The bf3 MLP backward kernel now stores pre-split bf16 triples in smaller per-wave LDS tiles so two workgroups fit per CU, removing redundant feature reloads and splits. These add tracking state and ordering subtleties (ticket reset, workspace zero invariants) in exchange for fewer launches, memsets and LDS/VGPR pressure.

After: 2.036 million, median of 2. About the same (-0.1%).

```diff
diff --git a/loner_amd/csrc/lnr_density.hip b/loner_amd/csrc/lnr_density.hip
--- a/loner_amd/csrc/lnr_density.hip
+++ b/loner_amd/csrc/lnr_density.hip
@@ -13,7 +13,7 @@
 #define LNR_ENC_BWD_MAX_BPG 2048
 
 namespace {
-struct WsNote { uint64_t layout; uint32_t epoch; bool ovf_zero; };
+struct WsNote { uint64_t layout; uint32_t epoch; bool ovf_zero; bool rayacc_zero; };
 std::mutex g_ws_mutex;
 std::unordered_map<const void*, WsNote> g_ws_notes;
 
@@ -29,14 +29,14 @@
     std::lock_guard<std::mutex> lock(g_ws_mutex);
     ws_bound_locked();
     auto it = g_ws_notes.find(ws);
-    if (it == g_ws_notes.end()) g_ws_notes[ws] = WsNote{layout, 0u, false};
-    else if (it->second.layout != layout) { it->second.layout = layout; it->second.ovf_zero = false; }
+    if (it == g_ws_notes.end()) g_ws_notes[ws] = WsNote{layout, 0u, false, false};
+    else if (it->second.layout != layout) { it->second.layout = layout; it->second.ovf_zero = false; it->second.rayacc_zero = false; }
 }
 void ws_backward_begin(const void* ws, uint64_t layout, int* epoch, bool* clear) {
     std::lock_guard<std::mutex> lock(g_ws_mutex);
     ws_bound_locked();
     WsNote& n = g_ws_notes[ws];
-    if (n.layout != layout) { n.layout = layout; n.ovf_zero = false; }
+    if (n.layout != layout) { n.layout = layout; n.ovf_zero = false; n.rayacc_zero = false; }
     *clear = !n.ovf_zero;
     n.ovf_zero = false;
     n.epoch = n.epoch >= 0x7FFFFFF0u ? 1u : n.epoch + 1u;
@@ -47,6 +47,20 @@
     std::lock_guard<std::mutex> lock(g_ws_mutex);
     auto it = g_ws_notes.find(ws);
     if (it != g_ws_notes.end()) it->second.ovf_zero = true;
+}
+bool ws_rayacc_begin(const void* ws, uint64_t layout) {
+    std::lock_guard<std::mutex> lock(g_ws_mutex);
+    ws_bound_locked();
+    WsNote& n = g_ws_notes[ws];
+    if (n.layout != layout) { n.layout = layout; n.ovf_zero = false; n.rayacc_zero = false; }
+    const bool clear = !n.rayacc_zero;
+    n.rayacc_zero = false;
+    return clear;
+}
+void ws_rayacc_done(const void* ws) {
+    std::lock_guard<std::mutex> lock(g_ws_mutex);
+    auto it = g_ws_notes.find(ws);
+    if (it != g_ws_notes.end()) it->second.rayacc_zero = true;
 }
 void ws_forget(const void* ws) {
     std::lock_guard<std::mutex> lock(g_ws_mutex);
@@ -250,11 +264,14 @@
     const uint32_t base = ((uint32_t)(lv.lo >> shift) + (uint32_t)local) << shift;
     const uint32_t region_bytes = plan.bytes[l];
     if (region_bytes == 0u) return;
+    const int per_part = (bpg + parts - 1) / parts, part_first = part * per_part, part_n = min(per_part, bpg - part_first);
+    int any = 0;
+    for (int i = threadIdx.x; i < part_n; i += 1024) any |= counts[((size_t)l * maxo + local) * bpg + part_first + i];
+    if (__syncthreads_or(any) == 0) return;
 #pragma unroll
     for (int i = threadIdx.x; i < slice; i += 1024) acc[i] = 0ll;
     __syncthreads();
     const int lane = threadIdx.x & 63, wave = __builtin_amdgcn_readfirstlane(threadIdx.x >> 6);
-    const int per_part = (bpg + parts - 1) / parts, part_first = part * per_part, part_n = min(per_part, bpg - part_first);
     const int per_wave = (part_n + 15) / 16, first = part_first + wave * per_wave, n_regions = min(per_wave, part_first + part_n - first);
     if (n_regions > 0)
         reduce_regions<PAIR, RED_U>(acc, counts + ((size_t)l * maxo + local) * bpg + first,
@@ -808,11 +825,18 @@
                    (flags & LNR_BWD_TABLE_ATOMICS) ? 0 : L.n_split, (flags & LNR_BWD_OVERWRITE_GRAD) ? 1 : 0,
                    fold_in_reduce ? slabs : nullptr, route.n_slabs, spec->n_mlp_params, grad_params};
     if (want_dfeat && !fused_freq) {
+        const bool rays_apply = ray_accum && hash;
+        if (rays_apply && ws_rayacc_begin(workspace, layout_signature(spec, cap)) &&
+            hipMemsetAsync(ws + L.off_rayacc, 0, L.off_slabs - L.off_rayacc, st) != hipSuccess) {
+            lnr_set_error("lnr_density_backward: hipMemsetAsync failed");
+            return LNR_ERR_LAUNCH;
+        }
         rc = lnr_encode_backward(spec, params, &src, cap, dfeat, dxl, L.m_pad, grad_table, want_grad ? regions : nullptr, &rplan, counts,
                                  L.bpg, L.maxo, L.shift,
                                  ovf, ovf_flag, epoch, d_pts_eff, ray_accum ? d_rays : nullptr, (long long*)(ws + L.off_rayacc), (flags & LNR_BWD_BINS_W8) != 0, st);
         if (rc) return rc;
         LNR_CHECK_LAUNCH("lnr_density_backward(encode backward)");
+        if (rays_apply) ws_rayacc_done(workspace);
     }
     if (d_rays && !ray_accum) {
         rc = lnr_points_grad_to_rays(d_pts_eff, z, n_rays, n_rays_dev, n_samples, d_rays, stream);
diff --git a/loner_amd/csrc/lnr_density_api.h b/loner_amd/csrc/lnr_density_api.h
--- a/loner_amd/csrc/lnr_density_api.h
+++ b/loner_amd/csrc/lnr_density_api.h
@@ -35,7 +35,9 @@
 #ifndef LNR_BATCHES_PER_WG
 #define LNR_BATCHES_PER_WG 4
 #endif
+#ifndef LNR_REDUCE_SPLIT
 #define LNR_REDUCE_SPLIT 32
+#endif
 #define LNR_FIX_SCALE 4398046511104.0f
 #define LNR_BIN_BYTES 1024
 #define LNR_BIN_MAX_OWNERS 64
diff --git a/loner_amd/csrc/lnr_density_bf3.hip b/loner_amd/csrc/lnr_density_bf3.hip
--- a/loner_amd/csrc/lnr_density_bf3.hip
+++ b/loner_amd/csrc/lnr_density_bf3.hip
@@ -3,7 +3,9 @@
 typedef __bf16 bf16x8 __attribute__((ext_vector_type(8)));
 typedef __bf16 bf16x2 __attribute__((ext_vector_type(2)));
 
-#define BF3_TS 36
+#define BF3_TS 20
+#define BF3_X_DWORDS (3 * 32 * BF3_TS)
+#define BF3_Z_DWORDS (3 * 16 * BF3_TS)
 #ifndef LNR_BF3_FWD_OCC
 #define LNR_BF3_FWD_OCC 3
 #endif
@@ -27,6 +29,10 @@
         bf3_split_pair(v[2 * q], v[2 * q + 1], p0, p1, p2);
         f.t[0][q] = p0; f.t[1][q] = p1; f.t[2][q] = p2;
     }
+}
+template <int H>
+__device__ __forceinline__ uint32_t bf3_halves(uint32_t k0, uint32_t k1) {
+    return __builtin_amdgcn_perm(k1, k0, H ? 0x07060302u : 0x05040100u);
 }
 #define BF3_M(a, b, acc) __builtin_amdgcn_mfma_f32_16x16x32_bf16(__builtin_bit_cast(bf16x8, a), __builtin_bit_cast(bf16x8, b), acc, 0, 0, 0)
 #define BF3_FOR_TERMS(X) X(0, 2) X(2, 0) X(1, 1) X(0, 1) X(1, 0) X(0, 0)
@@ -115,10 +121,12 @@
 struct Bf3Lds {
     static constexpr int H = 16 * HT, KB = (HT + 1) / 2, NW = LNR_DENSITY_BLOCK / 64;
     static constexpr size_t N_MLP = (size_t)H * 32 + 16 * H;
-    static constexpr size_t OFF_T = N_MLP * sizeof(float);
-    static constexpr size_t OFF_WA = OFF_T + (size_t)NW * H * BF3_TS * sizeof(float);
+    static constexpr size_t WAVE_DWORDS = BF3_X_DWORDS + BF3_Z_DWORDS;
+    static constexpr size_t OFF_WA = (size_t)NW * WAVE_DWORDS * sizeof(uint32_t);
     static constexpr size_t OFF_WT = OFF_WA + (size_t)3 * HT * 64 * 16;
     static constexpr size_t BYTES = OFF_WT + (size_t)3 * 2 * KB * 64 * 16;
+    static_assert(N_MLP * sizeof(float) <= OFF_WA, "dW lies over the tiles");
+    static_assert(2 * BYTES <= 160 * 1024, "two workgroups per CU");
 };
 
 template <int HT>
@@ -130,13 +138,13 @@
     using L = Bf3Lds<HT>;
     constexpr int H = 16 * HT, KB = L::KB;
     const int nw = blockDim.x >> 6;
-    const int lane = threadIdx.x & 63, wave = threadIdx.x >> 6;
+    const int lane = threadIdx.x & 63, wave = __builtin_amdgcn_readfirstlane(threadIdx.x >> 6);
     const int c = lane & 15, g = lane >> 4;
     float* dW = smem;
-    float* T = reinterpret_cast<float*>(reinterpret_cast<char*>(smem) + L::OFF_T) + wave * (H * BF3_TS);
+    uint32_t* XT = reinterpret_cast<uint32_t*>(smem) + wave * (int)L::WAVE_DWORDS;
+    uint32_t* ZT = XT + BF3_X_DWORDS;
     u32x4* WA = reinterpret_cast<u32x4*>(reinterpret_cast<char*>(smem) + L::OFF_WA);
     u32x4* WT = reinterpret_cast<u32x4*>(reinterpret_cast<char*>(smem) + L::OFF_WT);
-    for (int i = threadIdx.x; i < n_mlp; i += blockDim.x) dW[i] = 0.0f;
     for (int job = wave; job < HT + 2 * KB; job += nw) {
         float v[8];
         if (job < HT) {
@@ -178,14 +186,21 @@
     const int64_t n_tiles = M > 0 ? (M + 31) / 32 : 0;
     const int64_t stride = (int64_t)gridDim.x * nw;
     const uint32_t plane_bytes = (uint32_t)m_pad * 4u;
-    const float* fb = feat + (size_t)(8 * g) * m_pad;
-    const float* fc = feat + (size_t)c * m_pad;
-    float* db = dfeat + (size_t)(4 * g) * m_pad;
+    const uint32_t fb_off = (uint32_t)(8 * g) * plane_bytes;
+    const uint32_t db_off = (uint32_t)(4 * g) * plane_bytes;
+    uint32_t* xw = XT + (8 * g) * BF3_TS + c;
+    uint32_t* zw = ZT + (4 * g) * BF3_TS + c;
+    const u32x4* xr = reinterpret_cast<const u32x4*>(XT + c * BF3_TS + 4 * g);
+    const u32x4* zr = reinterpret_cast<const u32x4*>(ZT + c * BF3_TS + 4 * g);
     int64_t tile = (int64_t)blockIdx.x * nw + wave;
     float xcur[2][8], dcur[2];
     auto load_front = [&](int64_t tl, float (&x)[2][8], float (&ds)[2]) {
         const int64_t m = tl * 32 + 2 * c;
-        bf3_load_x2(fb, plane_bytes, (uint32_t)m, x);
+#pragma unroll
+        for (int i = 0; i < 8; ++i) {
+            const float2 v = ld32<float2>(feat, (uint32_t)i * plane_bytes + (fb_off + (uint32_t)m * 4u));
+            x[0][i] = v.x; x[1][i] = v.y;
+        }
         const float v0 = d_sigma[m < M ? m : M - 1], v1 = d_sigma[m + 1 < M ? m + 1 : M - 1];
         ds[0] = m < M ? v0 : 0.0f;
         ds[1] = m + 1 < M ? v1 : 0.0f;
@@ -202,20 +217,23 @@
             if (want_dfeat) {
 #pragma unroll
                 for (int k = 0; k < 8; ++k)
-                    st32<float2>(db, (uint32_t)(16 * (k >> 2) + (k & 3)) * plane_bytes + (uint32_t)(tile * 32 + 2 * c) * 4u, make_float2(0.0f, 0.0f));
+                    st32<float2>(dfeat, (uint32_t)(16 * (k >> 2) + (k & 3)) * plane_bytes + (db_off + (uint32_t)(tile * 32 + 2 * c) * 4u), make_float2(0.0f, 0.0f));
             }
         } else {
-            float xraw[2][8];
-#pragma unroll
-            for (int it = 0; it < 2; ++it) {
-                const uint32_t off = (uint32_t)(16 * it) * plane_bytes + (uint32_t)(tile * 32 + 8 * g) * 4u;
-                const float4 a = ld32<float4>(fc, off), b = ld32<float4>(fc, off + 16u);
-                xraw[it][0] = a.x; xraw[it][1] = a.y; xraw[it][2] = a.z; xraw[it][3] = a.w;
-                xraw[it][4] = b.x; xraw[it][5] = b.y; xraw[it][6] = b.z; xraw[it][7] = b.w;
-            }
             Frag3 xf[2];
-            bf3_split8(xcur[0], xf[0]);
-            bf3_split8(xcur[1], xf[1]);
+#pragma unroll
+            for (int q = 0; q < 4; ++q) {
+                uint32_t e[3], o[3];
+                bf3_split_pair(xcur[0][2 * q], xcur[1][2 * q], e[0], e[1], e[2]);
+                bf3_split_pair(xcur[0][2 * q + 1], xcur[1][2 * q + 1], o[0], o[1], o[2]);
+#pragma unroll
+                for (int t3 = 0; t3 < 3; ++t3) {
+                    xw[(t3 * 32 + 2 * q) * BF3_TS] = e[t3];
+                    xw[(t3 * 32 + 2 * q + 1) * BF3_TS] = o[t3];
+                    xf[0].t[t3][q] = bf3_halves<0>(e[t3], o[t3]);
+                    xf[1].t[t3][q] = bf3_halves<1>(e[t3], o[t3]);
+                }
+            }
             int wl = lane;
             asm volatile("" : "+v"(wl));
             float dz[HT][2][4];
@@ -231,34 +249,38 @@
 #pragma unroll
                 for (int r = 0; r < 4; ++r) {
                     dWo_acc[jt][r] += dcur[0] * fmaxf(Z0[r], 0.0f) + dcur[1] * fmaxf(Z1[r], 0.0f);
-                    dz[jt][0][r] = Z0[r] > 0.0f ? dcur[0] * wo[jt][r] : 0.0f;
-                    dz[jt][1][r] = Z1[r] > 0.0f ? dcur[1] * wo[jt][r] : 0.0f;
-                    *reinterpret_cast<float2*>(T + (16 * jt + 4 * g + r) * BF3_TS + 2 * c) = make_float2(dz[jt][0][r], dz[jt][1][r]);
+                    float w = wo[jt][r];
+                    asm volatile("" : "+v"(w));
+                    dz[jt][0][r] = Z0[r] > 0.0f ? dcur[0] * w : 0.0f;
+                    dz[jt][1][r] = Z1[r] > 0.0f ? dcur[1] * w : 0.0f;
                 }
             }
             Frag3 xs[2];
-            bf3_split8(xraw[0], xs[0]);
-            bf3_split8(xraw[1], xs[1]);
-#pragma unroll
-            for (int it = 0; it < 2; ++it)
-#pragma unroll
-                for (int t3 = 0; t3 < 3; ++t3) asm volatile("" : "+v"(xs[it].t[t3]));
-            if (want_dfeat) {
-                f32x4 D[2][2];
-#pragma unroll
-                for (int t = 0; t < 2; ++t) {
-                    D[t][0] = f32x4{0.0f, 0.0f, 0.0f, 0.0f}; D[t][1] = f32x4{0.0f, 0.0f, 0.0f, 0.0f};
-#pragma unroll
-                    for (int kb = 0; kb < KB; ++kb) {
-                        constexpr bool odd = (HT & 1) != 0;
-                        float v[8];
-#pragma unroll
-                        for (int i = 0; i < 4; ++i) {
-                            v[i] = dz[2 * kb][t][i];
-                            v[4 + i] = (odd && 2 * kb + 1 >= HT) ? 0.0f : dz[(2 * kb + 1 < HT) ? 2 * kb + 1 : 2 * kb][t][i];
-                        }
+            f32x4 D[2][2];
+#pragma unroll
+            for (int t = 0; t < 2; ++t) { D[t][0] = f32x4{0.0f, 0.0f, 0.0f, 0.0f}; D[t][1] = f32x4{0.0f, 0.0f, 0.0f, 0.0f}; }
+#pragma unroll
+            for (int kb = 0; kb < KB; ++kb) {
+                uint32_t P[2][4][3];
+#pragma unroll
+                for (int jl = 0; jl < 2; ++jl)
+#pragma unroll
+                    for (int r = 0; r < 4; ++r) {
+                        const int jt = 2 * kb + jl < HT ? 2 * kb + jl : HT - 1;
+                        if (2 * kb + jl < HT) bf3_split_pair(dz[jt][0][r], dz[jt][1][r], P[jl][r][0], P[jl][r][1], P[jl][r][2]);
+                        else P[jl][r][0] = P[jl][r][1] = P[jl][r][2] = 0u;
+                    }
+                if (want_dfeat) {
+#pragma unroll
+                    for (int t = 0; t < 2; ++t) {
                         Frag3 b;
-                        bf3_split8(v, b);
+#pragma unroll
+                        for (int t3 = 0; t3 < 3; ++t3)
+#pragma unroll
+                            for (int q = 0; q < 4; ++q) {
+                                const uint32_t k0 = P[q >> 1][2 * (q & 1)][t3], k1 = P[q >> 1][2 * (q & 1) + 1][t3];
+                                b.t[t3][q] = t ? bf3_halves<1>(k0, k1) : bf3_halves<0>(k0, k1);
+                            }
 #pragma unroll
                         for (int it = 0; it < 2; ++it) {
                             Frag3 a;
@@ -267,29 +289,42 @@
                             D[t][it] = bf3_mfma6(a, b, D[t][it]);
                         }
                     }
+                    if (kb == KB - 1) {
+#pragma unroll
+                        for (int it = 0; it < 2; ++it)
+#pragma unroll
+                            for (int r = 0; r < 4; ++r)
+                                st32<float2>(dfeat, (uint32_t)(16 * it + r) * plane_bytes + (db_off + (uint32_t)(tile * 32 + 2 * c) * 4u), make_float2(D[0][it][r], D[1][it][r]));
+                    }
                 }
 #pragma unroll
-                for (int it = 0; it < 2; ++it)
-#pragma unroll
-                    for (int r = 0; r < 4; ++r)
-                        st32<float2>(db, (uint32_t)(16 * it + r) * plane_bytes + (uint32_t)(tile * 32 + 2 * c) * 4u, make_float2(D[0][it][r], D[1][it][r]));
-            }
-            __builtin_amdgcn_fence(__ATOMIC_RELEASE, "wavefront");
-            __builtin_amdgcn_wave_barrier();
-            __builtin_amdgcn_fence(__ATOMIC_ACQUIRE, "wavefront");
-#pragma unroll
-            for (int jt = 0; jt < HT; ++jt) {
-                const float4 a0 = *reinterpret_cast<const float4*>(T + (16 * jt + c) * BF3_TS + 8 * g);
-                const float4 a1 = *reinterpret_cast<const float4*>(T + (16 * jt + c) * BF3_TS + 8 * g + 4);
-                const float v[8] = {a0.x, a0.y, a0.z, a0.w, a1.x, a1.y, a1.z, a1.w};
-                Frag3 a;
-                bf3_split8(v, a);
+                for (int jl = 0; jl < 2; ++jl) {
+                    const int jt = 2 * kb + jl < HT ? 2 * kb + jl : HT - 1;
+                    if (2 * kb + jl < HT) {
+#pragma unroll
+                        for (int r = 0; r < 4; ++r)
+#pragma unroll
+                            for (int t3 = 0; t3 < 3; ++t3) zw[(t3 * 16 + r) * BF3_TS] = P[jl][r][t3];
+                        __builtin_amdgcn_fence(__ATOMIC_RELEASE, "wavefront");
+                        __builtin_amdgcn_wave_barrier();
+                        __builtin_amdgcn_fence(__ATOMIC_ACQUIRE, "wavefront");
+                        Frag3 a;
+#pragma unroll
+                        for (int t3 = 0; t3 < 3; ++t3) a.t[t3] = zr[(t3 * 16 * BF3_TS) / 4];
+                        if (jl == 0) {
+#pragma unroll
+                            for (int it = 0; it < 2; ++it)
+#pragma unroll
+                                for (int t3 = 0; t3 < 3; ++t3) xs[it].t[t3] = xr[((t3 * 32 + 16 * it) * BF3_TS) / 4];
+                        }
 #define BF3_X(IA, IB) dW1_acc[jt][0] = BF3_M(a.t[IA], xs[0].t[IB], dW1_acc[jt][0]); dW1_acc[jt][1] = BF3_M(a.t[IA], xs[1].t[IB], dW1_acc[jt][1]);
-                BF3_FOR_TERMS(BF3_X)
+                        BF3_FOR_TERMS(BF3_X)
 #undef BF3_X
-            }
-            __builtin_amdgcn_fence(__ATOMIC_RELEASE, "wavefront");
-            __builtin_amdgcn_wave_barrier();
+                        __builtin_amdgcn_fence(__ATOMIC_RELEASE, "wavefront");
+                        __builtin_amdgcn_wave_barrier();
+                    }
+                }
+            }
         }
 #pragma unroll
         for (int t = 0; t < 2; ++t) {
@@ -299,6 +334,9 @@
         }
         tile = nt;
     }
+    __syncthreads();
+    for (int i = threadIdx.x; i < n_mlp; i += blockDim.x) dW[i] = 0.0f;
+    __syncthreads();
     float* dW1 = dW;
     float* dWo = dW + H * 32;
     for (int turn = 0; turn < nw; ++turn) {
diff --git a/loner_amd/csrc/lnr_encode.hip b/loner_amd/csrc/lnr_encode.hip
--- a/loner_amd/csrc/lnr_encode.hip
+++ b/loner_amd/csrc/lnr_encode.hip
@@ -365,12 +365,20 @@
 }
 
 __global__ void __launch_bounds__(ENC_BLOCK)
-ray_grad_apply_kernel(const long long* __restrict__ ray_acc, int n_rays, const int32_t* __restrict__ n_rays_dev, float* __restrict__ d_rays) {
-    const int i = blockIdx.x * ENC_BLOCK + threadIdx.x;
-    if (i >= lnr_live_rays(n_rays, n_rays_dev) * 6) return;
-    const long long q = ray_acc[i];
-    if (__builtin_expect(ray_acc[(size_t)n_rays * 6 + i / 6] != 0ll, 0)) d_rays[(size_t)(i / 6) * LNR_RAY_STRIDE + (i % 6)] = __builtin_nanf("");
-    else if (q != 0ll) d_rays[(size_t)(i / 6) * LNR_RAY_STRIDE + (i % 6)] += (float)((double)q * (1.0 / (double)LNR_FIX_SCALE));
+ray_grad_apply_kernel(long long* __restrict__ ray_acc, int n_rays, const int32_t* __restrict__ n_rays_dev, float* __restrict__ d_rays) {
+    const int ray = blockIdx.x * ENC_BLOCK + threadIdx.x;
+    if (ray >= lnr_live_rays(n_rays, n_rays_dev)) return;
+    long long* flag = ray_acc + (size_t)n_rays * 6 + ray;
+    const bool bad = *flag != 0ll;
+    if (__builtin_expect(bad, 0)) *flag = 0ll;
+#pragma unroll
+    for (int k = 0; k < 6; ++k) {
+        long long* a = ray_acc + (size_t)ray * 6 + k;
+        const long long q = *a;
+        if (q != 0ll) *a = 0ll;
+        if (__builtin_expect(bad, 0)) d_rays[(size_t)ray * LNR_RAY_STRIDE + k] = __builtin_nanf("");
+        else if (q != 0ll) d_rays[(size_t)ray * LNR_RAY_STRIDE + k] += (float)((double)q * (1.0 / (double)LNR_FIX_SCALE));
+    }
 }
 
 __device__ __forceinline__ void store_stream_b128(uint64_t global_addr, uint4 v) {
@@ -1061,10 +1069,6 @@
     const bool hash = spec->encoding == LNR_ENC_HASHGRID;
     const int dxm = d_rays_acc ? ENC_DX_RAYS : (d_pts ? ENC_DX_PLANES : ENC_DX_NONE);
     float* dx_out = d_rays_acc ? reinterpret_cast<float*>(ray_acc) : dxl;
-    if (d_rays_acc && hipMemsetAsync(ray_acc, 0, ((((size_t)src->n_rays * 7) * sizeof(long long)) + 15) & ~(size_t)15, st) != hipSuccess) {
-        lnr_set_error("lnr_density_backward: hipMemsetAsync failed");
-        return LNR_ERR_LAUNCH;
-    }
     int n_groups = 1;
     if (hash) n_groups = spec->n_levels;
     if (hash && (regions != nullptr || dxm != ENC_DX_NONE)) {
@@ -1171,7 +1175,7 @@
         hipLaunchKernelGGL(freq_backward_kernel, dim3((unsigned)blocks), dim3(ENC_BLOCK), 0, st, *spec, *src, dfeat, dxl, m_pad);
     }
     if (dxm == ENC_DX_RAYS) {
-        hipLaunchKernelGGL(ray_grad_apply_kernel, dim3((unsigned)((src->n_rays * 6 + ENC_BLOCK - 1) / ENC_BLOCK)), dim3(ENC_BLOCK), 0, st,
+        hipLaunchKernelGGL(ray_grad_apply_kernel, dim3((unsigned)((src->n_rays + ENC_BLOCK - 1) / ENC_BLOCK)), dim3(ENC_BLOCK), 0, st,
                            ray_acc, src->n_rays, src->n_rays_dev, d_rays_acc);
     }
     if (dxm == ENC_DX_PLANES) {
diff --git a/loner_amd/csrc/lnr_render.hip b/loner_amd/csrc/lnr_render.hip
--- a/loner_amd/csrc/lnr_render.hip
+++ b/loner_amd/csrc/lnr_render.hip
@@ -217,6 +217,22 @@
 }
 
 
+__device__ __forceinline__ void loss_reduce_block(const float* block_partials, int n_blocks, float* __restrict__ loss_out,
+                                                  int32_t* __restrict__ poison, int32_t poison_tag, float (*part)[8]) {
+    const int term = threadIdx.x & 7, slice = threadIdx.x >> 3;
+    float v = 0.0f;
+    if (term < 5)
+        for (int b = slice; b < n_blocks; b += 32) v += __hip_atomic_load(block_partials + (size_t)b * 8 + term, __ATOMIC_RELAXED, __HIP_MEMORY_SCOPE_AGENT);
+    v += __shfl_xor(v, 8, 64); v += __shfl_xor(v, 16, 64); v += __shfl_xor(v, 32, 64);
+    if ((threadIdx.x & 63) < 8) part[threadIdx.x >> 6][term] = v;
+    __syncthreads();
+    if (threadIdx.x < 5) {
+        const float t = loss_out[threadIdx.x] + (part[0][threadIdx.x] + part[1][threadIdx.x] + part[2][threadIdx.x] + part[3][threadIdx.x]);
+        loss_out[threadIdx.x] = t;
+        if (threadIdx.x == 0 && poison != nullptr && t != t && atomicCAS(poison, 0, LNR_POISON_NAN_LOSS) == 0) poison[1] = poison_tag;
+    }
+}
+
 template <int C>
 __global__ void __launch_bounds__(RENDER_BLOCK)
 los_loss_fused_kernel(const float* __restrict__ sigma, const float* __restrict__ z, const float* __restrict__ rays,
@@ -224,8 +240,10 @@
                       const float* __restrict__ noise, float noise_std, uint64_t seed, float scale, const LnrLossConfig cfg,
                       const int32_t* __restrict__ counts, float* __restrict__ loss_out, float* __restrict__ d_sigma,
                       float* __restrict__ d_rays, float* __restrict__ ray_stats, float* __restrict__ weights_out,
-                      float* __restrict__ block_partials, const float* __restrict__ far0_dev) {
-    __shared__ float s_terms[RAYS_PER_BLOCK][5];
+                      float* block_partials, const float* __restrict__ far0_dev, int32_t* __restrict__ poison, int32_t poison_tag) {
+    static_assert(RAYS_PER_BLOCK == 4, "the reduce is written for 256 threads and takes s_terms over as its part[4][8]");
+    __shared__ float s_terms[RAYS_PER_BLOCK][8];
+    __shared__ int s_last;
     const int lane = threadIdx.x & 63;
     const int ray = blockIdx.x * RAYS_PER_BLOCK + (threadIdx.x >> 6);
     const bool alive = ray < lnr_live_rays(n_rays, n_rays_dev);
@@ -234,30 +252,26 @@
         if (alive) los_loss_ray<C>(sigma, z, rays, depth_gt, S, noise, noise_std, seed, scale, cfg, counts, s_terms[threadIdx.x >> 6], false,
                                    d_sigma, d_rays, ray_stats, weights_out, ray, lane, far0_dev);
         __syncthreads();
-        if (threadIdx.x < 8) {
-            float v = 0.0f;
-            if (threadIdx.x < 5) for (int r = 0; r < RAYS_PER_BLOCK; ++r) v += s_terms[r][threadIdx.x];
-            block_partials[(size_t)blockIdx.x * 8 + threadIdx.x] = v;
+        uint32_t* ticket = reinterpret_cast<uint32_t*>(block_partials) + 7;
+        if (threadIdx.x < 64) {
+            if (threadIdx.x < 5) {
+                float v = 0.0f;
+                for (int r = 0; r < RAYS_PER_BLOCK; ++r) v += s_terms[r][threadIdx.x];
+                __hip_atomic_store(block_partials + (size_t)blockIdx.x * 8 + threadIdx.x, v, __ATOMIC_RELAXED, __HIP_MEMORY_SCOPE_AGENT);
+            }
+            __builtin_amdgcn_fence(__ATOMIC_RELEASE, "agent");
+            asm volatile("s_waitcnt vmcnt(0)" ::: "memory");
+            if (threadIdx.x == 0) s_last = __hip_atomic_fetch_add(ticket, 1u, __ATOMIC_RELAXED, __HIP_MEMORY_SCOPE_AGENT) == gridDim.x - 1u ? 1 : 0;
+        }
+        __syncthreads();
+        if (s_last) {
+            __builtin_amdgcn_fence(__ATOMIC_ACQUIRE, "agent");
+            loss_reduce_block(block_partials, (int)gridDim.x, loss_out, poison, poison_tag, s_terms);
+            if (threadIdx.x == 0) __hip_atomic_store(ticket, 0u, __ATOMIC_RELAXED, __HIP_MEMORY_SCOPE_AGENT);
         }
     } else if (alive) {
         los_loss_ray<C>(sigma, z, rays, depth_gt, S, noise, noise_std, seed, scale, cfg, counts, loss_out, true,
                         d_sigma, d_rays, ray_stats, weights_out, ray, lane, far0_dev);
-    }
-}
-
-__global__ void loss_reduce_kernel(const float* __restrict__ block_partials, int n_blocks, float* __restrict__ loss_out,
-                                   int32_t* __restrict__ poison, int32_t poison_tag) {
-    __shared__ float part[4][8];
-    const int term = threadIdx.x & 7, slice = threadIdx.x >> 3;
-    float v = 0.0f;
-    for (int b = slice; b < n_blocks; b += 32) v += block_partials[(size_t)b * 8 + term];
-    v += __shfl_xor(v, 8, 64); v += __shfl_xor(v, 16, 64); v += __shfl_xor(v, 32, 64);
-    if ((threadIdx.x & 63) < 8) part[threadIdx.x >> 6][term] = v;
-    __syncthreads();
-    if (threadIdx.x < 5) {
-        const float t = loss_out[threadIdx.x] + (part[0][threadIdx.x] + part[1][threadIdx.x] + part[2][threadIdx.x] + part[3][threadIdx.x]);
-        loss_out[threadIdx.x] = t;
-        if (threadIdx.x == 0 && poison != nullptr && t != t && atomicCAS(poison, 0, LNR_POISON_NAN_LOSS) == 0) poison[1] = poison_tag;
     }
 }
 
@@ -487,12 +501,8 @@
     hipStream_t st = (hipStream_t)stream;
     DISPATCH_C(n_samples, hipLaunchKernelGGL(los_loss_fused_kernel<C>, grid, block, 0, st, sigma, z, rays, depth_gt, n_rays, n_rays_dev,
                                              n_samples, noise, noise_std, seed, scale, *cfg, counts_dev, loss_out, d_sigma, d_rays,
-                                             ray_stats, weights_out, block_partials, far0_dev));
+                                             ray_stats, weights_out, block_partials, far0_dev, poison_dev, poison_tag));
     LNR_CHECK_LAUNCH("lnr_los_loss_fused");
-    if (block_partials) {
-        hipLaunchKernelGGL(loss_reduce_kernel, dim3(1), dim3(256), 0, st, block_partials, (int)grid.x, loss_out, poison_dev, poison_tag);
-        LNR_CHECK_LAUNCH("lnr_los_loss_fused(reduce)");
-    }
     return LNR_OK;
 }
 
diff --git a/loner_amd/ops.py b/loner_amd/ops.py
--- a/loner_amd/ops.py
+++ b/loner_amd/ops.py
@@ -691,6 +691,17 @@
     return counts
 
 
+_LOSS_PARTIALS = {}
+
+
+def _loss_partials(numel, dev):
+    key = (dev.index if dev.index is not None else torch.cuda.current_device(), _stream().value)
+    buf = _LOSS_PARTIALS.get(key)
+    if buf is None or buf.numel() < numel:
+        buf = _LOSS_PARTIALS[key] = torch.zeros(max(numel, 8192), device=dev)
+    return buf
+
+
 def los_loss_fused(sigma, z, rays, depth_gt, scale, cfg: hip.LossConfig, counts, noise=None, noise_std=0.0, seed=0,
                    n_rays_dev=None, want_stats=False, want_weights=False, loss_out=None, far0=None, poison=None, poison_tag=0,
                    zero_dead_rows=True):
@@ -704,7 +715,7 @@
     d_rays = (torch.zeros if (zero_dead_rows and n_rays_dev is not None) else torch.empty)(n, hip.RAY_STRIDE, device=dev)
     stats = torch.zeros(n, 8, device=dev) if want_stats else None
     w = torch.zeros(n, s, device=dev) if want_weights else None
-    partials = torch.empty(((n + hip.LOSS_RAYS_PER_BLOCK - 1) // hip.LOSS_RAYS_PER_BLOCK) * 8, device=dev)
+    partials = _loss_partials(((n + hip.LOSS_RAYS_PER_BLOCK - 1) // hip.LOSS_RAYS_PER_BLOCK) * 8, dev)
     check(load().lnr_los_loss_fused(_ptr(sigma), _ptr(z), _ptr(rays), _ptr(depth_gt), n, _ptr(n_rays_dev), s,
                                     _ptr(_f32c(noise)), float(noise_std), int(seed), float(scale), C.byref(cfg), _ptr(counts),
                                     _ptr(far0), _ptr(loss_out), _ptr(d_sigma), _ptr(d_rays), _ptr(stats), _ptr(w), _ptr(partials),
```
